# khaidoan25/prompt-tts

Hardware: NVIDIA B200
Metric: denoiser_train_codec_frames_per_sec (higher is better)
Workload: dtype bf16

## Files before the change

prompt_tts_b200/csrc/gemm_tcgen05.cu:

```cuda
#include <stdlib.h>

#include <mutex>

#include "tc_common.cuh"

namespace tc {
EncodeTiledFn get_encode_fn() {
  static EncodeTiledFn fn = nullptr;
  static std::once_flag once;
  std::call_once(once, [] {
    void* f = nullptr;
    cudaDriverEntryPointQueryResult qres;
    if (cudaGetDriverEntryPoint("cuTensorMapEncodeTiled", &f, cudaEnableDefault, &qres) == cudaSuccess && qres == cudaDriverEntryPointSuccess)
      fn = reinterpret_cast<EncodeTiledFn>(f);
  });
  return fn;
}
}

namespace {
using namespace tc;

constexpr int BM = 128;
constexpr int BK = 64;
constexpr int A_STAGE_BYTES = BM * BK * 2;

struct alignas(64) KParams {
  CUtensorMap tmA[2];
  CUtensorMap tmB[2];
  CUtensorMap tmO;
  pt_segment_t seg[8];
  int nseg;
  int a_kmajor, b_kmajor;
  int a_batched[2], b_batched[2];
  int M, N, nz2, nz3;
  int mt, nt, tiles, work, streamk;
  int gm;
  int total_iters;
  void* out;
  int out_dtype;
  long long osm, osz2, osz3;
  float alpha;
  const float* bias;
  const float* bias_z2;
  const bf16* res;
  long long rsm, rsz2, rsz3;
  long long bz2_stride;
  long long osn;
  int out_t;
  int vec_red;
};

template <int BN, bool PAIR = false>
struct Cfg {
  static constexpr int BN_LOAD = PAIR ? BN / 2 : BN;
  static constexpr int BN_S = (BN_LOAD + 63) / 64 * 64;
  static constexpr int B_STAGE_BYTES = BN_S * BK * 2;
  static constexpr int STAGE_BYTES = A_STAGE_BYTES + B_STAGE_BYTES;
  static constexpr int CTAS_PER_SM = (BN <= 128 && !PAIR) ? 2 : 1;
  static constexpr int EPI_WARPS = CTAS_PER_SM == 1 ? 8 : 4;
  static constexpr int EPI_SPLIT = EPI_WARPS / 4;
  static constexpr int THREADS = 64 + 32 * EPI_WARPS;
  static constexpr int EPI_COLS = 32;
#ifndef PT_EPI_BUFS
#define PT_EPI_BUFS 1
#endif
  static constexpr int EPI_BUFS = CTAS_PER_SM == 1 ? PT_EPI_BUFS : 1;
  static constexpr int EPI_BF16_BYTES = EPI_WARPS * EPI_BUFS * 32 * EPI_COLS * 2;
  static constexpr int EPI_F32_BYTES = EPI_WARPS * 32 * 17 * 4;
  static constexpr int EPI_BYTES = EPI_BF16_BYTES > EPI_F32_BYTES ? EPI_BF16_BYTES : EPI_F32_BYTES;
  static constexpr int F32_COLS = 16;
  static constexpr int BAR_BYTES = 512;
  static constexpr int BIAS_BYTES = 1024;
  static constexpr int AUX_BYTES = 1024  + BAR_BYTES + BIAS_BYTES + EPI_BYTES;
  static constexpr int STAGES_FIT = (227 * 1024 / CTAS_PER_SM - AUX_BYTES) / STAGE_BYTES;
  static constexpr int STAGES = STAGES_FIT > 8 ? 8 : STAGES_FIT;
  static constexpr int SMEM_BYTES = STAGES * STAGE_BYTES + AUX_BYTES;
  static constexpr int TMEM_COLS = 2 * BN <= 128 ? 128 : (2 * BN <= 256 ? 256 : 512);
};

struct Sched {
  int total_iters, streamk, cursor, end, stride;
  __device__ __forceinline__ Sched(const KParams& p, int mc) {
    total_iters = p.total_iters;
    streamk = p.streamk;
    const int nclu = (int)gridDim.x / mc, clu = (int)blockIdx.x / mc;
    if (streamk) {
      const int per = (p.work + nclu - 1) / nclu;
      cursor = min(p.work, clu * per);
      end = min(p.work, cursor + per);
      stride = 0;
    } else {
      cursor = clu;
      end = p.tiles;
      stride = nclu;
    }
  }
  __device__ __forceinline__ bool next(int& tile, int& it_begin, int& it_end) {
    if (cursor >= end) return false;
    if (streamk) {
      tile = cursor / total_iters;
      it_begin = cursor - tile * total_iters;
      it_end = min(total_iters, it_begin + (end - cursor));
      cursor += it_end - it_begin;
    } else {
      tile = cursor;
      it_begin = 0;
      it_end = total_iters;
      cursor += stride;
    }
    return true;
  }
};

template <int BN, int MC, bool PAIR>
__global__ void __launch_bounds__(Cfg<BN, PAIR>::THREADS, Cfg<BN, PAIR>::CTAS_PER_SM) gemm_kernel(const __grid_constant__ KParams p) {
  using C = Cfg<BN, PAIR>;
  static_assert(!PAIR || MC == 2, "a CTA pair is a cluster of two");
  const int crank = MC > 1 ? (int)cluster_ctarank() : 0;
  extern __shared__ uint8_t smem_raw[];
  const uint32_t smem_base = (smem_u32(smem_raw) + 1023u) & ~1023u;
  uint8_t* sgen = smem_raw + (smem_base - smem_u32(smem_raw));
  const uint32_t bar_base = smem_base + C::STAGES * C::STAGE_BYTES;
  auto full_bar = [&](int s) { return bar_base + 8u * s; };
  auto empty_bar = [&](int s) { return bar_base + 8u * (C::STAGES + s); };
  auto tmem_full_bar = [&](int a) { return bar_base + 8u * (2 * C::STAGES + a); };
  auto tmem_empty_bar = [&](int a) { return bar_base + 8u * (2 * C::STAGES + 2 + a); };
  const uint32_t tmem_slot = bar_base + 8u * (2 * C::STAGES + 4);
  float* sbias = reinterpret_cast<float*>(sgen + C::STAGES * C::STAGE_BYTES + C::BAR_BYTES);
  uint8_t* sepi = sgen + C::STAGES * C::STAGE_BYTES + C::BAR_BYTES + C::BIAS_BYTES;

  const int warp = threadIdx.x >> 5;
  const int lane = threadIdx.x & 31;

  if (warp == 0 && lane == 0) {
    asm volatile("prefetch.tensormap [%0];" ::"l"(reinterpret_cast<uint64_t>(&p.tmA[p.seg[0].a_idx])) : "memory");
    asm volatile("prefetch.tensormap [%0];" ::"l"(reinterpret_cast<uint64_t>(&p.tmB[p.seg[0].b_idx])) : "memory");
    for (int s = 0; s < C::STAGES; ++s) {
      mbar_init(full_bar(s), 1);
      mbar_init(empty_bar(s), PAIR ? 1 : MC);
    }
    for (int a = 0; a < 2; ++a) {
      mbar_init(tmem_full_bar(a), 1);
      mbar_init(tmem_empty_bar(a), PAIR ? 2 * C::EPI_WARPS : 32 * C::EPI_WARPS);
    }
    asm volatile("fence.mbarrier_init.release.cluster;" ::: "memory");
  }
  if (warp == 2) {
    if constexpr (PAIR) {
      asm volatile("tcgen05.alloc.cta_group::2.sync.aligned.shared::cta.b32 [%0], %1;" ::"r"(tmem_slot), "n"(C::TMEM_COLS) : "memory");
      asm volatile("tcgen05.relinquish_alloc_permit.cta_group::2.sync.aligned;" ::: "memory");
    } else {
      asm volatile("tcgen05.alloc.cta_group::1.sync.aligned.shared::cta.b32 [%0], %1;" ::"r"(tmem_slot), "n"(C::TMEM_COLS) : "memory");
      asm volatile("tcgen05.relinquish_alloc_permit.cta_group::1.sync.aligned;" ::: "memory");
    }
  }
  asm volatile("tcgen05.fence::before_thread_sync;" ::: "memory");
  __syncthreads();
  if (MC > 1) cluster_sync_all();
  asm volatile("tcgen05.fence::after_thread_sync;" ::: "memory");
  const uint32_t tmem_base = *reinterpret_cast<uint32_t*>(sgen + C::STAGES * C::STAGE_BYTES + 8 * (2 * C::STAGES + 4));

  auto decode = [&](int tile, int& m0, int& n0, int& z2, int& z3) {
    const int per_z = p.mt * p.nt;
    int r = tile / per_z;
    const int t = tile - r * per_z;
    const int span = p.gm * p.nt;
    const int grp = t / span;
    const int first = grp * p.gm;
    const int gsz = min(p.gm, p.mt - first);
    const int q = t - grp * span;
    const int mt = first + q % gsz;
    const int nt = q / gsz;
    m0 = (mt * MC + crank) * BM;
    n0 = nt * BN;
    z2 = r % p.nz2;
    z3 = r / p.nz2;
  };

  Sched sched(p, MC);
  int tile, it_begin, it_end;

  if (warp == 0) {
    const bool leader = elect_one();
    const uint32_t tx_own = A_STAGE_BYTES + (p.b_kmajor ? C::BN_LOAD * BK * 2 : C::B_STAGE_BYTES);
    const uint32_t tx_bytes = PAIR ? 2 * tx_own : tx_own;
    const uint32_t full0_leader = PAIR ? mapa_u32(full_bar(0), 0) : 0;
    int s = 0;
    uint32_t ph = 1;
    while (sched.next(tile, it_begin, it_end)) {
      int m0, n0, z2, z3;
      decode(tile, m0, n0, z2, z3);
      int seg = 0, rep = 0, kb = 0, skip = it_begin;
      while (true) {
        const int nkb = (p.seg[seg].nk + BK - 1) / BK;
        const int cnt = nkb * p.seg[seg].nrep;
        if (skip < cnt) {
          rep = skip / nkb;
          kb = skip % nkb;
          break;
        }
        skip -= cnt;
        ++seg;
      }
      for (int it = it_begin; it < it_end; ++it) {
        mbar_wait(empty_bar(s), ph);
        const pt_segment_t& sg = p.seg[seg];
        if (PAIR && leader) {
          if (crank == 0) mbar_expect_tx(full_bar(s), tx_bytes);
          const uint32_t sa = smem_base + s * C::STAGE_BYTES;
          const uint32_t sb = sa + A_STAGE_BYTES;
          const uint32_t fb = full0_leader + 8u * s;
          const CUtensorMap* ta = &p.tmA[sg.a_idx];
          const CUtensorMap* tb = &p.tmB[sg.b_idx];
          const int bz2 = sg.rep_is_batch ? (sg.rep_c2_0 + rep) : z2;
          const int a2 = p.a_batched[sg.a_idx] ? bz2 : 0, a3 = p.a_batched[sg.a_idx] ? z3 : 0;
          const int b2 = p.b_batched[sg.b_idx] ? bz2 : 0, b3 = p.b_batched[sg.b_idx] ? z3 : 0;
          const int ka = sg.a_k0 + kb * BK, kbb = sg.b_k0 + z2 * sg.b_k0_z2 + kb * BK;
          const int nb0 = n0 + sg.b_mn_shift + crank * C::BN_LOAD;
          if (p.a_kmajor) {
            tma_load_4d_pair(sa, ta, fb, ka, m0 + sg.a_mn_shift, a2, a3);
          } else {
#pragma unroll
            for (int j = 0; j < BM / 64; ++j) tma_load_4d_pair(sa + j * (BK * 128), ta, fb, m0 + sg.a_mn_shift + j * 64, ka, a2, a3);
          }
          if (p.b_kmajor) {
            tma_load_4d_pair(sb, tb, fb, kbb, nb0, b2, b3);
          } else {
#pragma unroll
            for (int j = 0; j < C::BN_S / 64; ++j) tma_load_4d_pair(sb + j * (BK * 128), tb, fb, nb0 + j * 64, kbb, b2, b3);
          }
        } else if (leader) {
          mbar_expect_tx(full_bar(s), tx_bytes);
          const uint32_t sa = smem_base + s * C::STAGE_BYTES;
          const uint32_t sb = sa + A_STAGE_BYTES;
          const CUtensorMap* ta = &p.tmA[sg.a_idx];
          const CUtensorMap* tb = &p.tmB[sg.b_idx];
          const int bz2 = sg.rep_is_batch ? (sg.rep_c2_0 + rep) : z2;
          const int a2 = p.a_batched[sg.a_idx] ? bz2 : 0, a3 = p.a_batched[sg.a_idx] ? z3 : 0;
          const int b2 = p.b_batched[sg.b_idx] ? bz2 : 0, b3 = p.b_batched[sg.b_idx] ? z3 : 0;
          const int ka = sg.a_k0 + kb * BK, kbb = sg.b_k0 + z2 * sg.b_k0_z2 + kb * BK;
          if (p.a_kmajor) {
            tma_load_4d(sa, ta, full_bar(s), ka, m0 + sg.a_mn_shift, a2, a3);
          } else {
#pragma unroll
            for (int j = 0; j < BM / 64; ++j) tma_load_4d(sa + j * (BK * 128), ta, full_bar(s), m0 + sg.a_mn_shift + j * 64, ka, a2, a3);
          }
          if (MC == 1) {
            if (p.b_kmajor) {
              tma_load_4d(sb, tb, full_bar(s), kbb, n0 + sg.b_mn_shift, b2, b3);
            } else {
#pragma unroll
              for (int j = 0; j < C::BN_S / 64; ++j) tma_load_4d(sb + j * (BK * 128), tb, full_bar(s), n0 + sg.b_mn_shift + j * 64, kbb, b2, b3);
            }
          } else {
            constexpr int HB = BN / MC;
            if (p.b_kmajor) {
              tma_load_4d_mc(sb + crank * (HB * 128), tb, full_bar(s), kbb, n0 + sg.b_mn_shift + crank * HB, b2, b3, (uint16_t)((1 << MC) - 1));
            } else {
#pragma unroll
              for (int j = 0; j < HB / 64; ++j) {
                const int jj = crank * (HB / 64) + j;
                tma_load_4d_mc(sb + jj * (BK * 128), tb, full_bar(s), n0 + sg.b_mn_shift + jj * 64, kbb, b2, b3, (uint16_t)((1 << MC) - 1));
              }
            }
          }
        }
        const int nkb = (sg.nk + BK - 1) / BK;
        if (++kb == nkb) {
          kb = 0;
          if (++rep == sg.nrep) {
            rep = 0;
            ++seg;
          }
        }
        if (++s == C::STAGES) s = 0, ph ^= 1;
      }
    }
  } else if (warp == 1 && (!PAIR || crank == 0)) {
    const bool leader = elect_one();
    const uint32_t idesc = idesc_f16(p.a_kmajor ? 0 : 1, p.b_kmajor ? 0 : 1, BN, PAIR ? 2 * BM : BM);
    const uint32_t a_lbo = p.a_kmajor ? 0u : (uint32_t)(BK * 128), b_lbo = p.b_kmajor ? 0u : (uint32_t)(BK * 128);
    const uint32_t a_kstep = p.a_kmajor ? 2u : 128u, b_kstep = p.b_kmajor ? 2u : 128u;
    const uint64_t adesc0 = umma_desc(smem_base, a_lbo, 1024);
    const uint64_t bdesc0 = umma_desc(smem_base + A_STAGE_BYTES, b_lbo, 1024);
    int s = 0;
    uint32_t ph = 0;
    int segi = 0;
    while (sched.next(tile, it_begin, it_end)) {
      const int acc = segi & 1;
      mbar_wait(tmem_empty_bar(acc), ((segi >> 1) & 1) ^ 1);
      asm volatile("tcgen05.fence::after_thread_sync;" ::: "memory");
      const uint32_t dcol = tmem_base + (uint32_t)(acc * BN);
      for (int it = it_begin; it < it_end; ++it) {
        mbar_wait(full_bar(s), ph);
        asm volatile("tcgen05.fence::after_thread_sync;" ::: "memory");
        if (leader) {
          const uint64_t ad = adesc0 + (uint64_t)(s * (C::STAGE_BYTES >> 4));
          const uint64_t bd = bdesc0 + (uint64_t)(s * (C::STAGE_BYTES >> 4));
          if constexpr (PAIR) {
#pragma unroll
            for (int k = 0; k < BK / 16; ++k)
              umma_f16_pair(dcol, ad + (uint64_t)(k * a_kstep), bd + (uint64_t)(k * b_kstep), idesc, (it > it_begin || k > 0) ? 1u : 0u);
            umma_commit_pair(empty_bar(s), (uint16_t)3);
            if (it == it_end - 1) umma_commit_pair(tmem_full_bar(acc), (uint16_t)3);
          } else {
#pragma unroll
            for (int k = 0; k < BK / 16; ++k)
              umma_f16(dcol, ad + (uint64_t)(k * a_kstep), bd + (uint64_t)(k * b_kstep), idesc, (it > it_begin || k > 0) ? 1u : 0u);
            if (MC == 1) umma_commit(empty_bar(s));
            else umma_commit_mc(empty_bar(s), (uint16_t)((1 << MC) - 1));
            if (it == it_end - 1) umma_commit(tmem_full_bar(acc));
          }
        }
        __syncwarp();
        if (++s == C::STAGES) s = 0, ph ^= 1;
      }
      ++segi;
    }
  } else if (warp >= 2) {
    const uint32_t tmem_empty_leader0 = PAIR ? mapa_u32(tmem_empty_bar(0), 0) : 0;
    auto release_acc = [&](int a) {
      asm volatile("tcgen05.fence::before_thread_sync;" ::: "memory");
      if constexpr (PAIR) {
        __syncwarp();
        if (lane == 0) mbar_arrive_cluster(tmem_empty_leader0 + 8u * a);
      } else {
        mbar_arrive(tmem_empty_bar(a));
      }
    };
    const int q = warp & 3;
    const int ew = warp - 2;
    const int half = ew >> 2;
    constexpr int ES = C::EPI_SPLIT;
    constexpr int ET = 32 * C::EPI_WARPS;
    const int et = threadIdx.x - 64;
    int segi = 0;
    int pc = 0;
    int staged_n0 = -1, staged_z2 = -1;
    while (sched.next(tile, it_begin, it_end)) {
      int m0, n0, z2, z3;
      decode(tile, m0, n0, z2, z3);
      const int acc = segi & 1;
      if (!p.out_t && (n0 != staged_n0 || (p.bias_z2 != nullptr && z2 != staged_z2))) {
        asm volatile("bar.sync 1, %0;" ::"n"(ET) : "memory");
        const float* bz = p.bias_z2 ? p.bias_z2 + (long long)z2 * p.bz2_stride : nullptr;
        for (int j = et; j < BN; j += ET) {
          const int n = n0 + j;
          float bsum = 0.f;
          if (n < p.N) {
            if (p.bias) bsum += __ldg(p.bias + n);
            if (bz) bsum += __ldg(bz + n);
          }
          sbias[j] = bsum;
        }
        asm volatile("bar.sync 1, %0;" ::"n"(ET) : "memory");
        staged_n0 = n0;
        staged_z2 = z2;
      }
      const uint32_t tbase = tmem_base + ((uint32_t)(q * 32) << 16) + (uint32_t)(acc * BN);
      const uint32_t full_parity = (segi >> 1) & 1;
      if (p.out_dtype == PT_OUT_BF16) {
        constexpr int CH = C::EPI_COLS;
        constexpr int NPASS = BN / CH;
        constexpr int NPH = (NPASS + ES - 1) / ES;
        constexpr int VPR = CH / 8;
        constexpr int RPI = 32 / VPR;
        constexpr int NIT = 32 / RPI;
        uint8_t* stg_base = sepi + ew * (C::EPI_BUFS * 32 * CH * 2);
        uint8_t* stg = stg_base + (pc & (C::EPI_BUFS - 1)) * (32 * CH * 2);
        auto cell = [&](int row, int chunk) { return stg + row * (CH * 2) + ((chunk ^ ((row >> 1) & 3)) << 4); };
        const int mw = m0 + q * 32;
        const int crow = lane / VPR, cvec = lane % VPR;
        const long long zoff_r = (long long)z2 * p.rsz2 + (long long)z3 * p.rsz3;
        const bool has_res = p.res != nullptr;
        const int last_c = min(NPASS, (p.N - n0 + CH - 1) / CH) - 1;
        const int last_k = last_c >= half ? (last_c - half) / ES : -1;
        uint32_t v[2][CH];
        bf16x8 rr[2][NIT];
        auto load_res = [&](int pass, bf16x8* dst) {
          if (p.out_t) {
            const int mb = mw + cvec * 8;
#pragma unroll
            for (int i = 0; i < NIT; ++i) {
              const int n = n0 + pass * CH + crow + i * RPI;
              if (n < p.N && mb < p.M) dst[i] = ld16(p.res + zoff_r + (long long)n * p.rsm + mb);
            }
            return;
          }
          const int nb = n0 + pass * CH + cvec * 8;
#pragma unroll
          for (int i = 0; i < NIT; ++i) {
            const int m = mw + crow + i * RPI;
            if (m < p.M && nb < p.N) dst[i] = ld16(p.res + zoff_r + (long long)m * p.rsm + nb);
          }
        };
        float brow = 0.f;
        if (p.out_t && mw + lane < p.M) {
          if (p.bias) brow += __ldg(p.bias + mw + lane);
          if (p.bias_z2) brow += __ldg(p.bias_z2 + (long long)z2 * p.bz2_stride + mw + lane);
        }
        if (has_res && last_k >= 0) load_res(half, rr[0]);
        mbar_wait(tmem_full_bar(acc), full_parity);
        asm volatile("tcgen05.fence::after_thread_sync;" ::: "memory");
        if (last_k < 0) {
          release_acc(acc);
        } else {
          tmem_ld32(tbase + (uint32_t)(half * CH), v[0]);
        }
#pragma unroll
        for (int k = 0; k < NPH; ++k) {
          const int c = half + k * ES;
          const int nb = n0 + c * CH;
          if (k <= last_k) {
            __syncwarp();
            asm volatile("tcgen05.wait::ld.sync.aligned;" ::: "memory");
            if (k < last_k) {
              tmem_ld32(tbase + (uint32_t)((c + ES) * CH), v[(k + 1) & 1]);
              if (has_res) load_res(c + ES, rr[(k + 1) & 1]);
            } else {
              release_acc(acc);
            }
            stg = stg_base + (pc & (C::EPI_BUFS - 1)) * (32 * CH * 2);
            if (lane == 0) {
              if (C::EPI_BUFS == 2) asm volatile("cp.async.bulk.wait_group.read 1;" ::: "memory");
              else asm volatile("cp.async.bulk.wait_group.read 0;" ::: "memory");
            }
            __syncwarp();
            if (has_res) {
#pragma unroll
              for (int i = 0; i < NIT; ++i) st16(cell(crow + i * RPI, cvec), rr[k & 1][i]);
              __syncwarp();
            }
            if (p.out_t) {
#pragma unroll
              for (int j = 0; j < CH; ++j) {
                bf16* cellp = reinterpret_cast<bf16*>(cell(j, lane >> 3)) + (lane & 7);
                float f = fmaf(__uint_as_float(v[k & 1][j]), p.alpha, brow);
                if (has_res) f += __bfloat162float(*cellp);
                *cellp = __float2bfloat16_rn(f);
              }
              fence_proxy_async_smem();
              __syncwarp();
              if (lane == 0) {
                tma_store_4d(&p.tmO, smem_u32(stg), mw, nb, z2, z3);
                tma_store_commit();
              }
              ++pc;
              continue;
            }
            const float* sb = sbias + c * CH;
#pragma unroll
            for (int g = 0; g < VPR; ++g) {
              const float4 b0 = *reinterpret_cast<const float4*>(sb + g * 8), b1 = *reinterpret_cast<const float4*>(sb + g * 8 + 4);
              const float bs[8] = {b0.x, b0.y, b0.z, b0.w, b1.x, b1.y, b1.z, b1.w};
              float f[8];
#pragma unroll
              for (int j = 0; j < 8; ++j) f[j] = fmaf(__uint_as_float(v[k & 1][g * 8 + j]), p.alpha, bs[j]);
              uint8_t* mine = cell(lane, g);
              if (has_res) {
                const bf16x8 t = ld16(mine);
#pragma unroll
                for (int h = 0; h < 4; ++h) {
                  const float2 u = bf2_to_f2(t.w[h]);
                  f[2 * h] += u.x;
                  f[2 * h + 1] += u.y;
                }
              }
              bf16x8 t;
#pragma unroll
              for (int h = 0; h < 4; ++h) t.w[h] = f2_to_bf2(f[2 * h], f[2 * h + 1]);
              st16(mine, t);
            }
            fence_proxy_async_smem();
            __syncwarp();
            if (lane == 0) {
              tma_store_4d(&p.tmO, smem_u32(stg), nb, mw, z2, z3);
              tma_store_commit();
            }
            ++pc;
          }
        }
      } else {
        const int m = m0 + q * 32 + lane;
        const bool m_ok = m < p.M;
        const long long out_off = (long long)z2 * p.osz2 + (long long)z3 * p.osz3 + (long long)m * p.osm;
        constexpr int FC = C::F32_COLS;
        constexpr int NCH = BN / FC;
        constexpr int NPH = (NCH + ES - 1) / ES;
        const int last_c = min(NCH, (p.N - n0 + FC - 1) / FC) - 1;
        const int last_k = last_c >= half ? (last_c - half) / ES : -1;
        uint32_t v[2][FC];
        mbar_wait(tmem_full_bar(acc), full_parity);
        asm volatile("tcgen05.fence::after_thread_sync;" ::: "memory");
        if (last_k < 0) {
          release_acc(acc);
        } else {
          tmem_ld16(tbase + (uint32_t)(half * FC), v[0]);
        }
        float* tile = reinterpret_cast<float*>(sepi) + ew * (32 * (FC + 1));
        const int mrow0 = m0 + q * 32;
        const long long zoff = (long long)z2 * p.osz2 + (long long)z3 * p.osz3;
#pragma unroll
        for (int k = 0; k < NPH; ++k) {
          const int c = half + k * ES;
          const int nb = n0 + c * FC;
          if (k <= last_k) {
            __syncwarp();
            asm volatile("tcgen05.wait::ld.sync.aligned;" ::: "memory");
            if (k < last_k) {
              tmem_ld16(tbase + (uint32_t)((c + ES) * FC), v[(k + 1) & 1]);
            } else {
              release_acc(acc);
            }
            float f[FC];
#pragma unroll
            for (int j = 0; j < FC; ++j) f[j] = fmaf(__uint_as_float(v[k & 1][j]), p.alpha, sbias[c * FC + j]);
            if (p.out_dtype == PT_OUT_F32) {
              if (m_ok) {
                float* o = reinterpret_cast<float*>(p.out) + out_off + nb;
#pragma unroll
                for (int g = 0; g < FC / 4; ++g) {
                  if (nb + g * 4 + 4 <= p.N) {
                    *reinterpret_cast<float4*>(o + g * 4) = make_float4(f[g * 4], f[g * 4 + 1], f[g * 4 + 2], f[g * 4 + 3]);
                  } else {
#pragma unroll
                    for (int j = 0; j < 4; ++j)
                      if (nb + g * 4 + j < p.N) o[g * 4 + j] = f[g * 4 + j];
                  }
                }
              }
            } else if (p.vec_red) {
              float* vt = reinterpret_cast<float*>(sepi) + ew * (32 * FC);
#pragma unroll
              for (int g = 0; g < FC / 4; ++g)
                *reinterpret_cast<float4*>(vt + lane * FC + ((g ^ ((lane >> 1) & 3)) << 2)) = make_float4(f[g * 4], f[g * 4 + 1], f[g * 4 + 2], f[g * 4 + 3]);
              __syncwarp();
              const int c4 = lane & 3, rsub = lane >> 2;
              const int n = nb + c4 * 4;
              if (n < p.N) {
                float* o = reinterpret_cast<float*>(p.out) + zoff + n;
#pragma unroll
                for (int it = 0; it < 4; ++it) {
                  const int r = it * 8 + rsub;
                  if (mrow0 + r < p.M) {
                    const float4 t = *reinterpret_cast<const float4*>(vt + r * FC + ((c4 ^ ((r >> 1) & 3)) << 2));
                    float* dst = o + (long long)(mrow0 + r) * p.osm;
                    if (n + 4 <= p.N) {
                      asm volatile("red.global.add.v4.f32 [%0], {%1, %2, %3, %4};" ::"l"(dst), "f"(t.x), "f"(t.y), "f"(t.z), "f"(t.w) : "memory");
                    } else {
                      const float tv[4] = {t.x, t.y, t.z, t.w};
#pragma unroll
                      for (int j = 0; j < 4; ++j)
                        if (n + j < p.N) atomicAdd(dst + j, tv[j]);
                    }
                  }
                }
              }
              __syncwarp();
            } else {
#pragma unroll
              for (int j = 0; j < FC; ++j) tile[lane * (FC + 1) + j] = f[j];
              __syncwarp();
              const int col = lane % FC, rsub = lane / FC;
              const int n = nb + col;
              if (n < p.N) {
                float* o = reinterpret_cast<float*>(p.out) + zoff + (long long)n * p.osn;
#pragma unroll 8
                for (int r = rsub; r < 32; r += 32 / FC) {
                  if (mrow0 + r < p.M) atomicAdd(o + (long long)(mrow0 + r) * p.osm, tile[r * (FC + 1) + col]);
                }
              }
            }
          }
        }
      }
      ++segi;
    }
    if (lane == 0) tma_store_wait_all();
  }

  asm volatile("tcgen05.fence::before_thread_sync;" ::: "memory");
  __syncthreads();
  if (MC > 1) cluster_sync_all();
  if (warp == 2) {
    if constexpr (PAIR) asm volatile("tcgen05.dealloc.cta_group::2.sync.aligned.b32 %0, %1;" ::"r"(tmem_base), "n"(C::TMEM_COLS) : "memory");
    else asm volatile("tcgen05.dealloc.cta_group::1.sync.aligned.b32 %0, %1;" ::"r"(tmem_base), "n"(C::TMEM_COLS) : "memory");
  }
}

int encode_operand(CUtensorMap* tm, const pt_operand_t& op, int box_rows_kmajor, const char* name) {
  EncodeTiledFn fn = get_encode_fn();
  if (!fn) {
    pt_set_error("cuTensorMapEncodeTiled not available from the driver");
    return PT_ECUDA;
  }
  PT_REQUIRE(op.ptr != nullptr, "gemm operand %s: null pointer", name);
  PT_REQUIRE((reinterpret_cast<uintptr_t>(op.ptr) & 15) == 0, "gemm operand %s: base not 16-byte aligned", name);
  PT_REQUIRE(op.stride[0] == 1, "gemm operand %s: dim[0] must be contiguous", name);
  cuuint64_t dims[4], strides[3];
  cuuint32_t box[4] = {64, 1, 1, 1}, estr[4] = {1, 1, 1, 1};
  for (int i = 0; i < 4; ++i) {
    PT_REQUIRE(op.dim[i] >= 1 && op.dim[i] < (1ll << 31), "gemm operand %s: dim[%d]=%lld out of range", name, i, (long long)op.dim[i]);
    dims[i] = (cuuint64_t)op.dim[i];
  }
  for (int i = 1; i < 4; ++i) {
    long long st = op.stride[i];
    if (op.dim[i] == 1 && (st <= 0 || (st % 8) != 0)) st = 8;
    PT_REQUIRE(st > 0 && st % 8 == 0, "gemm operand %s: stride[%d]=%lld must be a positive multiple of 8 elements", name, i, st);
    strides[i - 1] = (cuuint64_t)st * 2;
  }
  box[1] = op.kmajor ? (cuuint32_t)box_rows_kmajor : 64u;
  CUresult r = fn(tm, CU_TENSOR_MAP_DATA_TYPE_BFLOAT16, 4, const_cast<void*>(op.ptr), dims, strides, box, estr,
                  CU_TENSOR_MAP_INTERLEAVE_NONE, CU_TENSOR_MAP_SWIZZLE_128B, CU_TENSOR_MAP_L2_PROMOTION_L2_256B,
                  CU_TENSOR_MAP_FLOAT_OOB_FILL_NONE);
  if (r != CUDA_SUCCESS) {
    pt_set_error("cuTensorMapEncodeTiled(%s) failed: CUresult %d (dims %lld,%lld,%lld,%lld strides %lld,%lld,%lld box %u,%u)", name, (int)r,
                 (long long)dims[0], (long long)dims[1], (long long)dims[2], (long long)dims[3], (long long)strides[0],
                 (long long)strides[1], (long long)strides[2], box[0], box[1]);
    return PT_ECUDA;
  }
  return PT_OK;
}

int encode_output(CUtensorMap* tm, const pt_gemm_t* g) {
  EncodeTiledFn fn = get_encode_fn();
  if (!fn) {
    pt_set_error("cuTensorMapEncodeTiled not available from the driver");
    return PT_ECUDA;
  }
  PT_REQUIRE((reinterpret_cast<uintptr_t>(g->out) & 15) == 0, "pt_gemm: bf16 output base not 16-byte aligned");
  const long long ext[4] = {g->out_transposed ? g->M : g->N, g->out_transposed ? g->N : g->M, g->nz2, g->nz3};
  const long long str[4] = {1, g->out_stride_m, g->out_stride_z2, g->out_stride_z3};
  cuuint64_t dims[4], strides[3];
  for (int i = 0; i < 4; ++i) dims[i] = (cuuint64_t)ext[i];
  for (int i = 1; i < 4; ++i) {
    long long st = str[i];
    if (ext[i] == 1 && (st <= 0 || (st % 8) != 0)) st = 8;
    PT_REQUIRE(st > 0 && st % 8 == 0, "pt_gemm: bf16 output stride[%d]=%lld must be a positive multiple of 8 elements", i, st);
    strides[i - 1] = (cuuint64_t)st * 2;
  }
  cuuint32_t box[4] = {32, 32, 1, 1}, estr[4] = {1, 1, 1, 1};
  CUresult r = fn(tm, CU_TENSOR_MAP_DATA_TYPE_BFLOAT16, 4, g->out, dims, strides, box, estr, CU_TENSOR_MAP_INTERLEAVE_NONE,
                  CU_TENSOR_MAP_SWIZZLE_64B, CU_TENSOR_MAP_L2_PROMOTION_NONE, CU_TENSOR_MAP_FLOAT_OOB_FILL_NONE);
  if (r != CUDA_SUCCESS) {
    pt_set_error("cuTensorMapEncodeTiled(out) failed: CUresult %d (dims %lld,%lld,%lld,%lld strides %lld,%lld,%lld)", (int)r, ext[0], ext[1],
                 ext[2], ext[3], (long long)strides[0], (long long)strides[1], (long long)strides[2]);
    return PT_ECUDA;
  }
  return PT_OK;
}

template <int BN, int MC, bool PAIR = false>
int launch(const KParams& kp, dim3 grid, cudaStream_t st) {
  using CF = Cfg<BN, PAIR>;
  PT_ONCE_PER_DEVICE(cudaFuncSetAttribute(gemm_kernel<BN, MC, PAIR>, cudaFuncAttributeMaxDynamicSharedMemorySize, CF::SMEM_BYTES));
  if (MC == 1) {
    gemm_kernel<BN, MC, PAIR><<<grid, CF::THREADS, CF::SMEM_BYTES, st>>>(kp);
  } else {
    cudaLaunchConfig_t cfg = {};
    cfg.gridDim = grid;
    cfg.blockDim = dim3(CF::THREADS, 1, 1);
    cfg.dynamicSmemBytes = CF::SMEM_BYTES;
    cfg.stream = st;
    cudaLaunchAttribute attr[1];
    attr[0].id = cudaLaunchAttributeClusterDimension;
    attr[0].val.clusterDim.x = MC;
    attr[0].val.clusterDim.y = 1;
    attr[0].val.clusterDim.z = 1;
    cfg.attrs = attr;
    cfg.numAttrs = 1;
    static int max_clusters = 0;
    if (!max_clusters) {
      int n = 0;
      cudaLaunchConfig_t q = cfg;
      q.gridDim = dim3((unsigned)(pt_num_sms_physical() / MC * MC), 1, 1);
      if (cudaOccupancyMaxActiveClusters(&n, gemm_kernel<BN, MC, PAIR>, &q) != cudaSuccess || n < 1) {
        (void)cudaGetLastError();
        n = pt_num_sms_physical() / MC;
      }
      max_clusters = n;
      if (getenv("PT_GEMM_DEBUG")) fprintf(stderr, "[pt_gemm] BN=%d cluster=%d pair=%d: %d clusters resident at once\n", BN, MC, (int)PAIR, n);
    }
    if ((int)grid.x / MC > max_clusters) cfg.gridDim = dim3((unsigned)(max_clusters * MC), 1, 1);
    PT_CUDA_OK(cudaLaunchKernelEx(&cfg, gemm_kernel<BN, MC, PAIR>, kp));
  }
  PT_LAUNCH_CHECK();
  return PT_OK;
}

}

static thread_local int g_last_tile = 0;
extern "C" int pt_gemm_last_tile(void) { return g_last_tile; }

extern "C" int pt_gemm(const pt_gemm_t* g, void* stream) {
  PT_REQUIRE(g != nullptr, "pt_gemm: null descriptor");
  PT_REQUIRE(g->nseg >= 1 && g->nseg <= 8, "pt_gemm: nseg=%d", g->nseg);
  PT_REQUIRE(g->M >= 1 && g->N >= 1, "pt_gemm: M=%d N=%d", g->M, g->N);
  PT_REQUIRE(g->nz2 >= 1 && g->nz3 >= 1, "pt_gemm: bad batch extents");
  PT_REQUIRE(g->out != nullptr, "pt_gemm: null output");
  if (g->out_dtype == PT_OUT_BF16) {
    PT_REQUIRE((g->out_transposed ? g->M : g->N) % 8 == 0 && g->out_stride_m % 8 == 0 && g->out_stride_z2 % 8 == 0 && g->out_stride_z3 % 8 == 0 &&
                   (reinterpret_cast<uintptr_t>(g->out) & 15) == 0,
               "pt_gemm: bf16 output needs N (M if transposed), strides multiples of 8 and a 16-byte aligned base (M=%d N=%d)", g->M, g->N);
  } else if (g->out_dtype == PT_OUT_F32) {
    PT_REQUIRE(g->out_stride_m % 4 == 0 && g->out_stride_z2 % 4 == 0 && g->out_stride_z3 % 4 == 0 &&
                   (reinterpret_cast<uintptr_t>(g->out) & 15) == 0,
               "pt_gemm: f32 output needs N, strides multiples of 4 (N=%d)", g->N);
  } else {
    PT_REQUIRE(g->out_dtype == PT_OUT_F32_ATOMIC_ADD, "pt_gemm: out_dtype=%d", g->out_dtype);
  }
  if (g->residual) {
    PT_REQUIRE((g->out_transposed ? g->M : g->N) % 8 == 0 && g->res_stride_m % 8 == 0 && g->res_stride_z2 % 8 == 0 && g->res_stride_z3 % 8 == 0 &&
                   (reinterpret_cast<uintptr_t>(g->residual) & 15) == 0,
               "pt_gemm: residual alignment");
  }

  KParams kp;
  memset(&kp, 0, sizeof(kp));
  bool a_used[2] = {false, false}, b_used[2] = {false, false};
  long long total = 0;
  for (int i = 0; i < g->nseg; ++i) {
    const pt_segment_t& s = g->seg[i];
    PT_REQUIRE(s.a_idx >= 0 && s.a_idx < 2 && s.b_idx >= 0 && s.b_idx < 2, "pt_gemm: segment %d operand index", i);
    PT_REQUIRE(s.nk >= 1 && s.nrep >= 1, "pt_gemm: segment %d nk=%d nrep=%d", i, s.nk, s.nrep);
    a_used[s.a_idx] = true;
    b_used[s.b_idx] = true;
    kp.seg[i] = s;
    total += (long long)((s.nk + BK - 1) / BK) * s.nrep;
  }
  PT_REQUIRE(total < (1ll << 30), "pt_gemm: too many k iterations");
  const int a0 = a_used[0] ? 0 : 1, b0 = b_used[0] ? 0 : 1;
  kp.a_kmajor = g->a[a0].kmajor;
  kp.b_kmajor = g->b[b0].kmajor;
  for (int i = 0; i < 2; ++i) {
    if (a_used[i]) PT_REQUIRE(g->a[i].kmajor == kp.a_kmajor, "pt_gemm: A operands must share one majorness");
    if (b_used[i]) PT_REQUIRE(g->b[i].kmajor == kp.b_kmajor, "pt_gemm: B operands must share one majorness");
  }

  const bool streamk = g->out_dtype == PT_OUT_F32_ATOMIC_ADD;
  PT_REQUIRE(!streamk || (g->bias == nullptr && g->bias_z2 == nullptr && g->residual == nullptr),
             "pt_gemm: PT_OUT_F32_ATOMIC_ADD outputs are scheduled stream-K and take no bias/residual");
  int bn = g->block_n & ~1;
  bool table_no_cluster = false;
  const bool allow_cluster_arg = (g->block_n & 1) == 0;
  const long long mt = (g->M + BM - 1) / BM;
  const long long zz = (long long)g->nz2 * g->nz3;
  const int sms = pt_num_sms();
  if (g->block_n == 0) {
    struct TileRow { int M, N, K, zz, nseg, ak, bk, od, res, bn; };
    static const TileRow table[] = {
#include "gemm_tile_table.inc"
        {0, 0, 0, 0, 0, 0, 0, 0, 0, 0}};
    static const bool no_table = getenv("PT_GEMM_NO_TABLE") != nullptr;
    if (!no_table) {
      long long ktot = 0;
      for (int s = 0; s < g->nseg; ++s) ktot += (long long)g->seg[s].nk * g->seg[s].nrep;
      for (const TileRow& r : table)
        if (r.M == g->M && r.N == g->N && r.K == ktot && r.zz == zz && r.nseg == g->nseg && r.ak == kp.a_kmajor && r.bk == kp.b_kmajor &&
            r.od == g->out_dtype && r.res == (g->residual != nullptr)) {
          bn = r.bn & ~1;
          table_no_cluster = (r.bn & 1) != 0;
          break;
        }
    }
  }
  const bool allow_cluster = allow_cluster_arg && !table_no_cluster;
  if (bn == 0) {
    const int cand[6] = {256, 224, 192, 128, 64, 160};
    const double cyc[6] = {mt >= 2 && allow_cluster && !streamk ? 780.0 : 800.0, 730.0, 660.0, 430.0, streamk ? 416.0 : 260.0, 640.0};
    double best = 1e300;
    for (int i = 0; i < 6; ++i) {
      const int c = cand[i];
      const long long tiles_c = mt * ((g->N + c - 1) / c) * zz;
      double cost;
      if (streamk) {
        const double slots_c = (double)sms * (c <= 128 ? 2 : 1);
        cost = (double)tiles_c * (double)total * cyc[i] / sms + 0.65 * ((double)tiles_c + slots_c) * c;
      } else {
        cost = (double)((tiles_c + sms - 1) / sms) * ((double)total * cyc[i] + 500.0);
      }
      if (cost < best * 0.97) {
        best = cost;
        bn = c;
      }
    }
  }
  PT_REQUIRE(bn == 64 || bn == 96 || bn == 128 || bn == 160 || bn == 192 || bn == 224 || bn == 256, "pt_gemm: block_n=%d", bn);
  PT_REQUIRE(bn != 96 || kp.b_kmajor, "pt_gemm: block_n = 96 needs a K-major B operand");
  PT_REQUIRE(!g->out_transposed || (g->out_dtype == PT_OUT_BF16 && g->M % 8 == 0), "pt_gemm: out_transposed needs a bf16 output and M %% 8 == 0 (M=%d)", g->M);

  const int mc = (bn == 256 && mt >= 2 && allow_cluster && !streamk) ? 2 : 1;
  static const bool no_pair = getenv("PT_GEMM_NO_PAIR") != nullptr;
  const bool pair = mc == 2 && !no_pair && (mt % 2 == 0 || mt >= 8) && total >= 16;
  for (int i = 0; i < 2; ++i) {
    if (a_used[i]) {
      int r = encode_operand(&kp.tmA[i], g->a[i], BM, i ? "A1" : "A0");
      if (r) return r;
      kp.a_batched[i] = g->a[i].batched;
    }
    if (b_used[i]) {
      int r = encode_operand(&kp.tmB[i], g->b[i], bn / mc, i ? "B1" : "B0");
      if (r) return r;
      kp.b_batched[i] = g->b[i].batched;
    }
  }
  if (g->out_dtype == PT_OUT_BF16) {
    if (int r = encode_output(&kp.tmO, g)) return r;
  }
  kp.nseg = g->nseg;
  kp.M = g->M;
  kp.N = g->N;
  kp.nz2 = g->nz2;
  kp.nz3 = g->nz3;
  kp.total_iters = (int)total;
  const long long nt = (g->N + bn - 1) / bn;
  const long long mtg = (mt + mc - 1) / mc;
  const long long tiles = mtg * nt * zz;
  PT_REQUIRE(tiles * total < (1ll << 31), "pt_gemm: work space too large");
  kp.mt = (int)mtg;
  kp.nt = (int)nt;
  kp.tiles = (int)tiles;
  kp.work = (int)(tiles * total);
  kp.streamk = streamk ? 1 : 0;
  {
    static const bool no_group = getenv("PT_GEMM_NO_GROUP") != nullptr;
    const long long resident = (long long)sms * (bn <= 128 ? 2 : 1) / mc;
    long long gm = (resident + nt / 2) / nt;
    if (gm < 1) gm = 1;
    if (gm > mtg || no_group || streamk) gm = mtg;
    kp.gm = (int)gm;
  }
  kp.out = g->out;
  kp.out_dtype = g->out_dtype;
  kp.osm = g->out_stride_m;
  kp.osz2 = g->out_stride_z2;
  kp.osz3 = g->out_stride_z3;
  kp.alpha = g->alpha;
  kp.bias = g->bias;
  kp.bias_z2 = g->bias_z2;
  kp.res = reinterpret_cast<const bf16*>(g->residual);
  kp.rsm = g->res_stride_m;
  kp.rsz2 = g->res_stride_z2;
  kp.rsz3 = g->res_stride_z3;
  kp.bz2_stride = g->bias_z2_stride ? g->bias_z2_stride : g->N;
  kp.osn = g->out_stride_n ? g->out_stride_n : 1;
  kp.out_t = g->out_transposed ? 1 : 0;
  PT_REQUIRE(kp.osn == 1 || g->out_dtype == PT_OUT_F32_ATOMIC_ADD, "pt_gemm: out_stride_n needs PT_OUT_F32_ATOMIC_ADD");
  kp.vec_red = (g->out_dtype == PT_OUT_F32_ATOMIC_ADD && kp.osn == 1 && g->out_stride_m % 4 == 0 && g->out_stride_z2 % 4 == 0 &&
                g->out_stride_z3 % 4 == 0 && (reinterpret_cast<uintptr_t>(g->out) & 15) == 0 && !getenv("PT_GEMM_SCALAR_RED"))
                   ? 1 : 0;

  const long long slots = (long long)sms * (bn <= 128 ? 2 : 1) / mc;
  long long G = streamk ? (kp.work / 4 > 0 ? kp.work / 4 : 1) : tiles;
  if (G > slots) G = slots;
  dim3 grid((unsigned)(G * mc), 1, 1);
  cudaStream_t st = reinterpret_cast<cudaStream_t>(stream);
  g_last_tile = bn | (bn == 256 && mc == 1 ? 1 : 0);
  switch (bn) {
    case 64: return launch<64, 1>(kp, grid, st);
    case 96: return launch<96, 1>(kp, grid, st);
    case 128: return launch<128, 1>(kp, grid, st);
    case 160: return launch<160, 1>(kp, grid, st);
    case 192: return launch<192, 1>(kp, grid, st);
    case 224: return launch<224, 1>(kp, grid, st);
    default: return mc == 2 ? (pair ? launch<256, 2, true>(kp, grid, st) : launch<256, 2>(kp, grid, st)) : launch<256, 1>(kp, grid, st);
  }
}
```

prompt_tts_b200/csrc/tc_common.cuh:

```cuda
#pragma once
#include <cuda.h>

#include "common.cuh"

namespace tc {

__device__ __forceinline__ uint32_t smem_u32(const void* p) { return (uint32_t)__cvta_generic_to_shared(p); }

__device__ __forceinline__ bool elect_one() {
  uint32_t pred;
  asm volatile(
      "{\n\t.reg .pred p;\n\t"
      "elect.sync _|p, 0xffffffff;\n\t"
      "selp.u32 %0, 1, 0, p;\n\t}"
      : "=r"(pred));
  return pred != 0;
}

__device__ __forceinline__ void mbar_init(uint32_t bar, uint32_t count) {
  asm volatile("mbarrier.init.shared::cta.b64 [%0], %1;" ::"r"(bar), "r"(count) : "memory");
}
__device__ __forceinline__ void mbar_arrive(uint32_t bar) {
  asm volatile("mbarrier.arrive.shared::cta.b64 _, [%0];" ::"r"(bar) : "memory");
}
__device__ __forceinline__ void mbar_expect_tx(uint32_t bar, uint32_t bytes) {
  asm volatile("mbarrier.arrive.expect_tx.shared::cta.b64 _, [%0], %1;" ::"r"(bar), "r"(bytes) : "memory");
}
__device__ __forceinline__ void mbar_wait(uint32_t bar, uint32_t parity) {
  uint32_t done = 0;
  uint32_t spins = 0;
  while (true) {
    asm volatile(
        "{\n\t.reg .pred p;\n\t"
        "mbarrier.try_wait.parity.shared::cta.b64 p, [%1], %2;\n\t"
        "selp.u32 %0, 1, 0, p;\n\t}"
        : "=r"(done)
        : "r"(bar), "r"(parity)
        : "memory");
    if (done) break;
#ifdef PT_MBAR_WATCH
    if (spins == (1u << 20)) PT_MBAR_WATCH(bar, parity);
#endif
    if (++spins > (1u << 22)) __trap();
  }
}

__device__ __forceinline__ void tma_load_4d(uint32_t dst, const CUtensorMap* tm, uint32_t bar, int c0, int c1, int c2, int c3) {
  asm volatile(
      "cp.async.bulk.tensor.4d.shared::cluster.global.mbarrier::complete_tx::bytes [%0], [%1, {%3, %4, %5, %6}], [%2];"
      ::"r"(dst), "l"(reinterpret_cast<uint64_t>(tm)), "r"(bar), "r"(c0), "r"(c1), "r"(c2), "r"(c3)
      : "memory");
}

__device__ __forceinline__ void tma_store_4d(const CUtensorMap* tm, uint32_t src, int c0, int c1, int c2, int c3) {
  asm volatile("cp.async.bulk.tensor.4d.global.shared::cta.bulk_group [%0, {%2, %3, %4, %5}], [%1];" ::"l"(reinterpret_cast<uint64_t>(tm)),
               "r"(src), "r"(c0), "r"(c1), "r"(c2), "r"(c3)
               : "memory");
}
__device__ __forceinline__ void tma_store_commit() { asm volatile("cp.async.bulk.commit_group;" ::: "memory"); }
__device__ __forceinline__ void tma_store_wait_read() { asm volatile("cp.async.bulk.wait_group.read 0;" ::: "memory"); }
__device__ __forceinline__ void tma_store_wait_all() { asm volatile("cp.async.bulk.wait_group 0;" ::: "memory"); }
__device__ __forceinline__ void fence_proxy_async_smem() { asm volatile("fence.proxy.async.shared::cta;" ::: "memory"); }

__device__ __forceinline__ void tma_load_4d_mc(uint32_t dst, const CUtensorMap* tm, uint32_t bar, int c0, int c1, int c2, int c3, uint16_t mask) {
  asm volatile(
      "cp.async.bulk.tensor.4d.shared::cluster.global.mbarrier::complete_tx::bytes.multicast::cluster [%0], [%1, {%3, %4, %5, %6}], [%2], %7;"
      ::"r"(dst), "l"(reinterpret_cast<uint64_t>(tm)), "r"(bar), "r"(c0), "r"(c1), "r"(c2), "r"(c3), "h"(mask)
      : "memory");
}

__device__ __forceinline__ uint64_t umma_desc(uint32_t saddr, uint32_t lbo_bytes, uint32_t sbo_bytes) {
  uint64_t d = 0;
  d |= (uint64_t)((saddr >> 4) & 0x3FFF);
  d |= (uint64_t)((lbo_bytes >> 4) & 0x3FFF) << 16;
  d |= (uint64_t)((sbo_bytes >> 4) & 0x3FFF) << 32;
  d |= 1ull << 46;
  d |= 2ull << 61;
  return d;
}

__device__ __forceinline__ void umma_f16(uint32_t tmem_d, uint64_t adesc, uint64_t bdesc, uint32_t idesc, uint32_t accumulate) {
  asm volatile(
      "{\n\t.reg .pred p;\n\t"
      "setp.ne.b32 p, %4, 0;\n\t"
      "tcgen05.mma.cta_group::1.kind::f16 [%0], %1, %2, %3, p;\n\t}"
      ::"r"(tmem_d), "l"(adesc), "l"(bdesc), "r"(idesc), "r"(accumulate)
      : "memory");
}
__device__ __forceinline__ void umma_f16_ts(uint32_t tmem_d, uint32_t tmem_a, uint64_t bdesc, uint32_t idesc, uint32_t accumulate) {
  asm volatile(
      "{\n\t.reg .pred p;\n\t"
      "setp.ne.b32 p, %4, 0;\n\t"
      "tcgen05.mma.cta_group::1.kind::f16 [%0], [%1], %2, %3, p;\n\t}"
      ::"r"(tmem_d), "r"(tmem_a), "l"(bdesc), "r"(idesc), "r"(accumulate)
      : "memory");
}
__device__ __forceinline__ void umma_commit(uint32_t bar) {
  asm volatile("tcgen05.commit.cta_group::1.mbarrier::arrive::one.shared::cluster.b64 [%0];" ::"r"(bar) : "memory");
}

__device__ __forceinline__ void umma_commit_mc(uint32_t bar, uint16_t mask) {
  asm volatile("tcgen05.commit.cta_group::1.mbarrier::arrive::one.shared::cluster.multicast::cluster.b64 [%0], %1;" ::"r"(bar), "h"(mask) : "memory");
}
__device__ __forceinline__ uint32_t mapa_u32(uint32_t addr, uint32_t rank) {
  uint32_t r;
  asm volatile("mapa.shared::cluster.u32 %0, %1, %2;" : "=r"(r) : "r"(addr), "r"(rank));
  return r;
}
__device__ __forceinline__ void tma_load_4d_pair(uint32_t dst, const CUtensorMap* tm, uint32_t bar_cluster, int c0, int c1, int c2, int c3) {
  asm volatile(
      "cp.async.bulk.tensor.4d.cta_group::2.shared::cluster.global.mbarrier::complete_tx::bytes [%0], [%1, {%3, %4, %5, %6}], [%2];"
      ::"r"(dst), "l"(reinterpret_cast<uint64_t>(tm)), "r"(bar_cluster), "r"(c0), "r"(c1), "r"(c2), "r"(c3)
      : "memory");
}
__device__ __forceinline__ void mbar_arrive_cluster(uint32_t bar_cluster) {
  asm volatile("mbarrier.arrive.release.cluster.shared::cluster.b64 _, [%0];" ::"r"(bar_cluster) : "memory");
}
__device__ __forceinline__ void umma_f16_pair(uint32_t tmem_d, uint64_t adesc, uint64_t bdesc, uint32_t idesc, uint32_t accumulate) {
  asm volatile(
      "{\n\t.reg .pred p;\n\t"
      "setp.ne.b32 p, %4, 0;\n\t"
      "tcgen05.mma.cta_group::2.kind::f16 [%0], %1, %2, %3, p;\n\t}"
      ::"r"(tmem_d), "l"(adesc), "l"(bdesc), "r"(idesc), "r"(accumulate)
      : "memory");
}
__device__ __forceinline__ void umma_commit_pair(uint32_t bar, uint16_t mask) {
  asm volatile("tcgen05.commit.cta_group::2.mbarrier::arrive::one.shared::cluster.multicast::cluster.b64 [%0], %1;" ::"r"(bar), "h"(mask) : "memory");
}

__device__ __forceinline__ uint32_t cluster_ctarank() {
  uint32_t r;
  asm volatile("mov.u32 %0, %%cluster_ctarank;" : "=r"(r));
  return r;
}
__device__ __forceinline__ void cluster_sync_all() {
  asm volatile("barrier.cluster.arrive.release.aligned;" ::: "memory");
  asm volatile("barrier.cluster.wait.acquire.aligned;" ::: "memory");
}

__device__ __forceinline__ void tmem_st16(uint32_t taddr, const uint32_t* v) {
  asm volatile(
      "tcgen05.st.sync.aligned.32x32b.x16.b32 [%0], "
      "{%1, %2, %3, %4, %5, %6, %7, %8, %9, %10, %11, %12, %13, %14, %15, %16};"
      ::"r"(taddr), "r"(v[0]), "r"(v[1]), "r"(v[2]), "r"(v[3]), "r"(v[4]), "r"(v[5]), "r"(v[6]), "r"(v[7]), "r"(v[8]), "r"(v[9]), "r"(v[10]),
        "r"(v[11]), "r"(v[12]), "r"(v[13]), "r"(v[14]), "r"(v[15])
      : "memory");
}
__device__ __forceinline__ void tmem_wait_st() { asm volatile("tcgen05.wait::st.sync.aligned;" ::: "memory"); }

__device__ __forceinline__ void tmem_ld32(uint32_t taddr, uint32_t* v) {
  asm volatile(
      "tcgen05.ld.sync.aligned.32x32b.x32.b32 "
      "{%0, %1, %2, %3, %4, %5, %6, %7, %8, %9, %10, %11, %12, %13, %14, %15, "
      "%16, %17, %18, %19, %20, %21, %22, %23, %24, %25, %26, %27, %28, %29, %30, %31}, [%32];"
      : "=r"(v[0]), "=r"(v[1]), "=r"(v[2]), "=r"(v[3]), "=r"(v[4]), "=r"(v[5]), "=r"(v[6]), "=r"(v[7]), "=r"(v[8]),
        "=r"(v[9]), "=r"(v[10]), "=r"(v[11]), "=r"(v[12]), "=r"(v[13]), "=r"(v[14]), "=r"(v[15]), "=r"(v[16]),
        "=r"(v[17]), "=r"(v[18]), "=r"(v[19]), "=r"(v[20]), "=r"(v[21]), "=r"(v[22]), "=r"(v[23]), "=r"(v[24]),
        "=r"(v[25]), "=r"(v[26]), "=r"(v[27]), "=r"(v[28]), "=r"(v[29]), "=r"(v[30]), "=r"(v[31])
      : "r"(taddr)
      : "memory");
}
__device__ __forceinline__ void tmem_ld16(uint32_t taddr, uint32_t* v) {
  asm volatile(
      "tcgen05.ld.sync.aligned.32x32b.x16.b32 "
      "{%0, %1, %2, %3, %4, %5, %6, %7, %8, %9, %10, %11, %12, %13, %14, %15}, [%16];"
      : "=r"(v[0]), "=r"(v[1]), "=r"(v[2]), "=r"(v[3]), "=r"(v[4]), "=r"(v[5]), "=r"(v[6]), "=r"(v[7]), "=r"(v[8]),
        "=r"(v[9]), "=r"(v[10]), "=r"(v[11]), "=r"(v[12]), "=r"(v[13]), "=r"(v[14]), "=r"(v[15])
      : "r"(taddr)
      : "memory");
}

__device__ __forceinline__ uint32_t idesc_f16(int a_mn_major, int b_mn_major, int n, int m) {
  return (1u << 4) | (1u << 7) | (1u << 10) | ((uint32_t)a_mn_major << 15) | ((uint32_t)b_mn_major << 16) | ((uint32_t)(n >> 3) << 17) |
         ((uint32_t)(m >> 4) << 24);
}

typedef CUresult (*EncodeTiledFn)(CUtensorMap*, CUtensorMapDataType, cuuint32_t, void*, const cuuint64_t*, const cuuint64_t*,
                                  const cuuint32_t*, const cuuint32_t*, CUtensorMapInterleave, CUtensorMapSwizzle,
                                  CUtensorMapL2promotion, CUtensorMapFloatOOBfill);
EncodeTiledFn get_encode_fn();

}
```

prompt_tts_b200/engine.py:

```python
from __future__ import annotations

import os
from typing import Callable, Dict, List, Optional, Sequence, Tuple

import torch

from . import ops
from .ops import BF16, F32, OUT_BF16, OUT_F32, OUT_F32_ATOMIC_ADD



class Var:
    __slots__ = ("data", "grad", "owned", "needs_grad")

    def __init__(self, data: torch.Tensor, needs_grad: bool = True):
        self.data = data
        self.grad: Optional[torch.Tensor] = None
        self.owned = False
        self.needs_grad = needs_grad


class SideLane:

    def __init__(self, device):
        self.stream = torch.cuda.Stream(device)
        self.keep: List[torch.Tensor] = []
        self.dirty = False

    def run(self, fn: Callable[[], None], keep: Sequence[torch.Tensor] = ()) -> None:
        self.stream.wait_stream(torch.cuda.current_stream())
        with torch.cuda.stream(self.stream):
            fn()
        self.keep.extend(keep)
        self.dirty = True

    def join(self) -> None:
        if self.dirty:
            torch.cuda.current_stream().wait_stream(self.stream)
            self.dirty = False
            self.keep.clear()


SIDE_LANE = os.environ.get("PT_SIDE_LANE", "0") == "1"


class PackCache:

    def __init__(self):
        self._d: Dict[tuple, Tuple[tuple, torch.Tensor]] = {}
        self.static: Dict[tuple, list] = {}
        self.lane: Optional[SideLane] = None
        self.epoch = 0

    def add_static(self, kind: str, params: Sequence[torch.Tensor], view: torch.Tensor, refresh: Optional[Callable[[], None]]) -> None:
        key = (kind,) + tuple(id(p) for p in params)
        self.static[key] = [tuple(p._version for p in params), view, refresh, list(params)]

    def get(self, params: Sequence[torch.Tensor], kind: str) -> torch.Tensor:
        key = (kind,) + tuple(id(p) for p in params)
        st = self.static.get(key)
        if st is not None:
            ver = tuple(p._version for p in params)
            if ver != st[0]:
                if st[2] is not None:
                    st[2]()
                st[0] = ver
            return st[1]
        ver = (self.epoch,) + tuple((p._version, p.data_ptr()) for p in params)
        hit = self._d.get(key)
        capturing = torch.cuda.is_current_stream_capturing() if params[0].is_cuda else False
        if hit is not None and hit[0] == ver and not capturing:
            return hit[1]
        prev = hit[1] if hit is not None else None
        if kind == "conv":
            (w,) = params
            if not w.is_contiguous():
                raise ops._lib.PtError("conv weight is a non-contiguous view (optimiser-managed) but has no static bf16 shadow")
            out = ops.pack_conv_weight(w.detach(), out=prev)
        elif kind == "bias":
            if len(params) == 1:
                out = params[0].detach()
            else:
                out = torch.cat([p.detach() for p in params], out=prev) if prev is not None else torch.cat([p.detach() for p in params])
        else:
            rows = sum(p.shape[0] for p in params)
            K = params[0].numel() // params[0].shape[0]
            out = prev if prev is not None else torch.empty(rows, K, dtype=BF16, device=params[0].device)
            r = 0
            for p in params:
                ops.cast_bf16(p.detach().reshape(p.shape[0], K), out[r:r + p.shape[0]])
                r += p.shape[0]
        self._d[key] = (ver, out)
        return out


class Tape:
    def __init__(self, cache: PackCache, recording: bool = True):
        self.cache = cache
        self.recording = recording
        self.bwd: List[Callable[[], None]] = []
        self.pgrads: Dict[int, torch.Tensor] = {}
        self.params: Dict[int, torch.Tensor] = {}
        self.post: List[Callable[[], None]] = []
        self.pgrad_order: List[Tuple[Sequence[torch.Tensor], torch.Tensor, str]] = []
        self.grad_alloc: Optional[Callable[[Sequence[torch.Tensor], str], Optional[torch.Tensor]]] = None
        self.on_ready: Optional[Callable[[List[Tuple[Sequence[torch.Tensor], torch.Tensor, str]]], None]] = None
        self.kv_cache: Optional[Dict[int, "Var"]] = None
        self.kv_group: Dict[int, Tuple["Var", int, int]] = {}

    def record(self, fn: Callable[[], None]) -> None:
        if self.recording:
            self.bwd.append(fn)

    def _register(self, params: Sequence[torch.Tensor], kind: str, buf: torch.Tensor) -> None:
        if kind == "plain":
            (p,) = params
            self.pgrads[id(p)] = buf.view(p.shape)
            self.params[id(p)] = p
        elif kind == "conv":
            (p,) = params
            Co, Ci, k = p.shape
            packed = buf.view(Co, k, Ci)
            g = packed.permute(0, 2, 1)
            g._pt_buf = packed
            self.pgrads[id(p)] = g
            self.params[id(p)] = p
        else:
            rows = sum(p.shape[0] for p in params)
            K = params[0].numel() // params[0].shape[0]
            cat = buf.view(rows, K)
            r = 0
            for p in params:
                v = cat[r:r + p.shape[0]].view(p.shape)
                v._pt_buf = cat
                self.pgrads[id(p)] = v
                self.params[id(p)] = p
                r += p.shape[0]

    def _grad_buf(self, params: Sequence[torch.Tensor], kind: str) -> torch.Tensor:
        g = self.pgrads.get(id(params[0]))
        if g is None:
            n = sum(p.numel() for p in params)
            buf = self.grad_alloc(params, kind) if self.grad_alloc is not None else None
            if buf is None:
                buf = torch.zeros(n, dtype=F32, device=params[0].device)
            self._register(params, kind, buf)
            self.pgrad_order.append((list(params), buf, kind))
            g = self.pgrads[id(params[0])]
        return getattr(g, "_pt_buf", g)

    def rebind(self, params: Sequence[torch.Tensor], kind: str, buf: torch.Tensor) -> None:
        self._register(params, kind, buf)

    def pgrad(self, p: torch.Tensor) -> torch.Tensor:
        return self._grad_buf([p], "plain")

    def pgrad_cat(self, params: Sequence[torch.Tensor]) -> torch.Tensor:
        return self._grad_buf(params, "cat")

    def pgrad_conv(self, p: torch.Tensor) -> torch.Tensor:
        return self._grad_buf([p], "conv")

    def side_colsum(self, x2d: torch.Tensor, out: torch.Tensor) -> None:
        if not SIDE_LANE or not x2d.is_cuda:
            ops.colsum(x2d, out)
            return
        if self.cache.lane is None:
            self.cache.lane = SideLane(x2d.device)
        self.cache.lane.run(lambda: ops.colsum(x2d, out, lite=True), keep=(x2d, out))

    def join_side(self) -> None:
        if self.cache.lane is not None:
            self.cache.lane.join()

    def backward(self) -> None:
        done = 0
        for fn in reversed(self.bwd):
            fn()
            if self.on_ready is not None and len(self.pgrad_order) > done:
                self.on_ready(self.pgrad_order[done:])
                done = len(self.pgrad_order)
        self.bwd = []
        self.join_side()
        for fn in self.post:
            fn()
        self.post = []


def accum(v: Var, g: torch.Tensor, owned: bool = True) -> None:
    if not v.needs_grad:
        return
    if v.grad is None:
        v.grad, v.owned = g, owned
    elif v.owned:
        ops.add_(v.grad, g, out=v.grad)
    else:
        v.grad = ops.add_(v.grad, g)
        v.owned = True


def _wgrad_gemm(dy2d_op, x2d_op, seg, N: int, K: int, out: torch.Tensor, out_stride_m: int) -> None:
    ops.gemm([dy2d_op], [x2d_op], [seg], N, K, out, out_strides=(out_stride_m, 0, 0), out_mode=OUT_F32_ATOMIC_ADD)


def linear(tape: Tape, x: Var, wparams: Sequence[torch.Tensor], bias: Optional[Sequence[torch.Tensor]] = None,
           residual: Optional[Var] = None, out_f32: bool = False) -> Var:
    xd = x.data
    K = xd.shape[-1]
    x2 = xd.reshape(-1, K)
    M = x2.shape[0]
    wp = tape.cache.get(wparams, "lin")
    N = wp.shape[0]
    out = torch.empty(xd.shape[:-1] + (N,), dtype=F32 if out_f32 else BF16, device=xd.device)
    res = residual.data.reshape(M, N) if residual is not None else None
    ops.gemm([ops.operand(x2, True)], [ops.operand(wp, True)], [ops.segment(K)], M, N, out,
             out_mode=OUT_F32 if out_f32 else OUT_BF16, bias=tape.cache.get(bias, "bias") if bias is not None else None, residual=res)
    y = Var(out)

    def bwd():
        dy = y.grad
        if dy is None:
            return
        if out_f32:
            dy = ops.cast_bf16(dy)
        dy2 = dy.reshape(M, N)
        if bias is not None:
            tape.side_colsum(dy2, tape.pgrad_cat(bias) if len(bias) > 1 else tape.pgrad(bias[0]))
        gw = (tape.pgrad_cat(wparams) if len(wparams) > 1 else tape.pgrad(wparams[0])).view(N, K)
        _wgrad_gemm(ops.operand(dy2, False), ops.operand(x2, False), ops.segment(M), N, K, gw, K)
        if x.needs_grad:
            dx = torch.empty_like(x2) if (x.grad is None or not x.owned) else x.grad.reshape(M, K)
            prev = x.grad.reshape(M, K) if x.grad is not None else None
            ops.gemm([ops.operand(dy2, True)], [ops.operand(wp, False)], [ops.segment(N)], M, K, dx, residual=prev)
            x.grad, x.owned = dx.view(xd.shape), True
        if residual is not None:
            accum(residual, dy.view(residual.data.shape) if not out_f32 else dy.view(residual.data.shape), owned=False)

    tape.record(bwd)
    return y


class TimeShift:

    def __init__(self, proj: torch.Tensor, dproj: Optional[torch.Tensor], offset: int):
        self.proj, self.dproj, self.offset = proj, dproj, offset


CONV_SWAP = os.environ.get("PT_CONV_NO_SWAP") is None


def _swap_tile(L: int, rows: int) -> int:
    if not CONV_SWAP or rows % 128 != 0 or L > 96:
        return 0
    bn = 64 if L <= 64 else 96
    return bn if L / bn > L / 128 + 0.08 else 0


def conv3(tape: Tape, x: Var, wparam: torch.Tensor, bias: torch.Tensor, stride: int = 1,
          tshift: Optional[TimeShift] = None, residual: Optional[Var] = None) -> Var:
    xd = x.data
    B, L, Ci = xd.shape
    wp = tape.cache.get([wparam], "conv")
    Co = wp.shape[0]
    Lo = L if stride == 1 else (L - 1) // 2 + 1
    out = torch.empty(B, Lo, Co, dtype=BF16, device=xd.device)
    if stride == 1:
        a_ops = [ops.operand(xd, True, batched=True)]
        taps = [(0, t - 1) for t in range(3)]
    else:
        a_ops = [ops.operand(xd[:, 0::2], True, batched=True), ops.operand(xd[:, 1::2], True, batched=True)]
        taps = [(1, -1), (0, 0), (1, 0)]
    segs = [ops.segment(Ci, a_idx=ai, a_shift=sh, b_k0=t * Ci) for t, (ai, sh) in enumerate(taps)]
    bz2 = tshift.proj[:, tshift.offset:] if tshift is not None else None
    sw = _swap_tile(L, Co) if stride == 1 else 0
    if sw:
        segs_w = [ops.segment(Ci, a_k0=t * Ci, b_shift=t - 1) for t in range(3)]
        ops.gemm([ops.operand(wp, True)], a_ops, segs_w, Co, Lo, out, out_strides=(Co, Lo * Co, 0), nz2=B,
                 bias=bias.detach(), bias_z2=bz2, bias_z2_stride=tshift.proj.stride(0) if tshift is not None else 0,
                 residual=residual.data if residual is not None else None, res_strides=(Co, Lo * Co, 0), block_n=sw, out_transposed=True)
    else:
        ops.gemm(a_ops, [ops.operand(wp, True)], segs, Lo, Co, out, out_strides=(Co, Lo * Co, 0), nz2=B,
                 bias=bias.detach(), bias_z2=bz2, bias_z2_stride=tshift.proj.stride(0) if tshift is not None else 0,
                 residual=residual.data if residual is not None else None, res_strides=(Co, Lo * Co, 0))
    y = Var(out)

    def bwd():
        dy = y.grad
        if dy is None:
            return
        tape.side_colsum(dy.view(B * Lo, Co), tape.pgrad(bias))
        if tshift is not None and tshift.dproj is not None:
            ops.batch_colsum(dy, tshift.dproj[:, tshift.offset:], tshift.dproj.stride(0))
        g3 = tape.pgrad_conv(wparam)
        dy_op = ops.operand(dy, False, batched=True)
        if stride == 1:
            seg = ops.segment(Lo, b_k0=-1, b_k0_z2=1, nrep=B, rep_is_batch=True)
            ops.gemm([dy_op], [ops.operand(xd, False, batched=True)], [seg], Co, Ci, g3, out_strides=(3 * Ci, Ci, 0), nz2=3,
                     out_mode=OUT_F32_ATOMIC_ADD)
        else:
            for t, (ai, sh) in enumerate(taps):
                xs = xd[:, 0::2] if ai == 0 else xd[:, 1::2]
                seg = ops.segment(Lo, b_k0=sh, nrep=B, rep_is_batch=True)
                ops.gemm([dy_op], [ops.operand(xs, False, batched=True)], [seg], Co, Ci, g3[:, t],
                         out_strides=(3 * Ci, 0, 0), out_mode=OUT_F32_ATOMIC_ADD)
        if x.needs_grad:
            dy_k = ops.operand(dy, True, batched=True)
            wp_mn = ops.operand(wp, False)
            if stride == 1:
                own = x.grad is not None and x.owned
                dx = x.grad if own else torch.empty_like(xd)
                swx = _swap_tile(L, Ci)
                if swx:
                    segs_dx = [ops.segment(Co, a_shift=t * Ci, b_shift=1 - t) for t in range(3)]
                    ops.gemm([wp_mn], [dy_k], segs_dx, Ci, L, dx, out_strides=(Ci, L * Ci, 0), nz2=B,
                             residual=x.grad, res_strides=(Ci, L * Ci, 0), block_n=swx, out_transposed=True)
                else:
                    segs_dx = [ops.segment(Co, a_shift=1 - t, b_shift=t * Ci) for t in range(3)]
                    ops.gemm([dy_k], [wp_mn], segs_dx, L, Ci, dx, out_strides=(Ci, L * Ci, 0), nz2=B,
                             residual=x.grad, res_strides=(Ci, L * Ci, 0))
                x.grad, x.owned = dx, True
            else:
                dx = torch.empty_like(xd)
                ev, od = dx[:, 0::2], dx[:, 1::2]
                ops.gemm([dy_k], [wp_mn], [ops.segment(Co, b_shift=Ci)], ev.shape[1], Ci, ev, out_strides=(2 * Ci, L * Ci, 0), nz2=B)
                if od.shape[1] > 0:
                    ops.gemm([dy_k], [wp_mn], [ops.segment(Co, a_shift=1, b_shift=0), ops.segment(Co, a_shift=0, b_shift=2 * Ci)],
                             od.shape[1], Ci, od, out_strides=(2 * Ci, L * Ci, 0), nz2=B)
                accum(x, dx, owned=True)
        if residual is not None:
            accum(residual, dy, owned=False)

    tape.record(bwd)
    return y


def groupnorm(tape: Tape, x: Var, gamma: torch.Tensor, beta: torch.Tensor, eps: float, act: bool, groups: int = 32) -> Var:
    yd, stats = ops.groupnorm_fwd(x.data, gamma.detach(), beta.detach(), groups, eps, act)
    y = Var(yd)

    def bwd():
        if y.grad is None:
            return
        if not x.needs_grad:
            ops.groupnorm_bwd(y.grad, x.data, stats, gamma.detach(), beta.detach(), tape.pgrad(gamma), tape.pgrad(beta), groups, act)
            return
        prev = x.grad
        dx = ops.groupnorm_bwd(y.grad, x.data, stats, gamma.detach(), beta.detach(), tape.pgrad(gamma), tape.pgrad(beta), groups, act,
                               dx_add=prev, out=prev if (prev is not None and x.owned) else None)
        x.grad, x.owned = dx, True

    tape.record(bwd)
    return y


def layernorm(tape: Tape, x: Var, gamma: torch.Tensor, beta: torch.Tensor, eps: float = 1e-5) -> Var:
    xd = x.data
    Cc = xd.shape[-1]
    x2 = xd.reshape(-1, Cc)
    yd, rs = ops.layernorm_fwd(x2, gamma.detach(), beta.detach(), eps)
    y = Var(yd.view(xd.shape))

    def bwd():
        if y.grad is None:
            return
        prev = x.grad.reshape(-1, Cc) if x.grad is not None else None
        dx = ops.layernorm_bwd(y.grad.reshape(-1, Cc), x2, rs, gamma.detach(), tape.pgrad(gamma), tape.pgrad(beta), dx_add=prev)
        if x.needs_grad:
            x.grad, x.owned = dx.view(xd.shape), True

    tape.record(bwd)
    return y


def attention_core(tape: Tape, q_src: Var, q_off: int, kv_src: Var, k_off: int, v_off: int, heads: int, C: int,
                   shared_kv: bool = False) -> Var:
    qd, kvd = q_src.data, kv_src.data
    B, Lq, _ = qd.shape
    d = C // heads
    scale = d ** -0.5
    qv, kv_, vv = qd[:, :, q_off:q_off + C], kvd[:, :, k_off:k_off + C], kvd[:, :, v_off:v_off + C]
    o = torch.empty(B, Lq, C, dtype=BF16, device=qd.device)
    lse = torch.empty(B, heads, Lq, dtype=F32, device=qd.device)
    ops.attn_fwd(qv, kv_, vv, o, lse, heads, d, scale)
    y = Var(o)

    def bwd():
        do = y.grad
        if do is None:
            return
        same = q_src is kv_src
        dq_buf = torch.empty_like(qd)
        if shared_kv:
            if kv_src.grad is None:
                kv_src.grad, kv_src.owned = torch.empty_like(kvd), True
            dkv_buf = kv_src.grad
        else:
            dkv_buf = dq_buf if same else torch.empty_like(kvd)
        ops.attn_bwd(qv, kv_, vv, o, lse, do, dq_buf[:, :, q_off:q_off + C], dkv_buf[:, :, k_off:k_off + C],
                     dkv_buf[:, :, v_off:v_off + C], heads, d, scale)
        accum(q_src, dq_buf, owned=True)
        if not same and not shared_kv:
            accum(kv_src, dkv_buf, owned=True)

    tape.record(bwd)
    return y


def geglu(tape: Tape, u: Var) -> Var:
    ud = u.data
    u2 = ud.reshape(-1, ud.shape[-1])
    y = Var(ops.geglu_fwd(u2).view(ud.shape[:-1] + (ud.shape[-1] // 2,)))

    def bwd():
        if y.grad is None:
            return
        accum(u, ops.geglu_bwd(y.grad.reshape(-1, ud.shape[-1] // 2), u2).view(ud.shape), owned=True)

    tape.record(bwd)
    return y


def add(tape: Tape, a: Var, b: Var) -> Var:
    y = Var(ops.add_(a.data, b.data))

    def bwd():
        if y.grad is None:
            return
        accum(a, y.grad, owned=False)
        accum(b, y.grad, owned=False)

    tape.record(bwd)
    return y


def concat_channels(tape: Tape, a: Var, b: Var) -> Var:
    B, L, Ca = a.data.shape
    Cb = b.data.shape[2]
    out = torch.empty(B, L, Ca + Cb, dtype=BF16, device=a.data.device)
    ops.copy2d(a.data, Ca, out, Ca + Cb, B * L, Ca)
    ops.copy2d(b.data, Cb, out[:, :, Ca:], Ca + Cb, B * L, Cb)
    y = Var(out)

    def bwd():
        if y.grad is None:
            return
        g = y.grad
        ga = torch.empty_like(a.data)
        gb = torch.empty_like(b.data)
        ops.copy2d(g, Ca + Cb, ga, Ca, B * L, Ca)
        ops.copy2d(g[:, :, Ca:], Ca + Cb, gb, Cb, B * L, Cb)
        accum(a, ga, owned=True)
        accum(b, gb, owned=True)

    tape.record(bwd)
    return y


def upsample2(tape: Tape, x: Var) -> Var:
    y = Var(ops.upsample2_fwd(x.data))

    def bwd():
        if y.grad is None:
            return
        accum(x, ops.upsample2_bwd(y.grad), owned=True)

    tape.record(bwd)
    return y


def silu_f32(tape: Tape, x: Var) -> Var:
    y = Var(ops.silu_to_bf16(x.data))

    def bwd():
        if y.grad is None or not x.needs_grad:
            return
        g = ops.silu_bwd(x.data, ops.cast_f32(y.grad))
        if x.grad is None:
            x.grad, x.owned = g, True
        else:
            x.grad = x.grad + g

    tape.record(bwd)
    return y


class TapeFunction(torch.autograd.Function):

    @staticmethod
    def forward(ctx, runner, cache, n_in, *args):
        ins, params = args[:n_in], args[n_in:]
        need = any(ctx.needs_input_grad[3:])
        tape = Tape(cache, recording=need)
        outs, seed, in_grads = runner(tape, *ins)
        ctx.tape, ctx.seed, ctx.in_grads, ctx.n_in, ctx.params = tape, seed, in_grads, n_in, params
        ctx.mark_non_differentiable(*[o for o in outs if not o.is_floating_point()])
        return outs if len(outs) > 1 else outs[0]

    @staticmethod
    def backward(ctx, *gouts):
        tape = ctx.tape
        ctx.seed([g.contiguous() if g is not None else None for g in gouts])
        tape.backward()
        gin = ctx.in_grads()
        gparams = tuple(tape.pgrads.get(id(p)) if ctx.needs_input_grad[3 + ctx.n_in + i] else None for i, p in enumerate(ctx.params))
        ctx.tape = None
        return (None, None, None) + tuple(gin) + gparams


def get_cache(module) -> PackCache:
    c = module.__dict__.get("_pt_pack_cache")
    if c is None:
        c = PackCache()
        module.__dict__["_pt_pack_cache"] = c
    return c


def run_module(module, body, inputs, kinds, out_kind="ncl", multi=False):
    params = [p for p in module.parameters()]
    cache = get_cache(module)
    for t in inputs:
        if not t.is_cuda:
            raise ops._lib.PtError(f"{type(module).__name__}: inputs must be CUDA tensors; there is no CPU fallback")

    def runner(tape, *ins):
        vs = []
        for t, k in zip(ins, kinds):
            if k == "ncl":
                vs.append(Var(ops.ncl_to_nlc(t.detach().float().contiguous())))
            elif k == "blc":
                vs.append(Var(ops.cast_bf16(t.detach().float().contiguous())))
            elif k == "f32":
                vs.append(Var(t.detach().float().contiguous()))
            else:
                vs.append(t.detach())
        res = body(tape, *vs)
        yvs = list(res) if multi else [res]
        outs = tuple(ops.nlc_to_ncl(v.data) if out_kind == "ncl" else ops.cast_f32(v.data) for v in yvs)

        def seed(gouts):
            for v, g in zip(yvs, gouts):
                if g is None:
                    continue
                gg = ops.ncl_to_nlc(g.float().contiguous()) if out_kind == "ncl" else ops.cast_bf16(g.float().contiguous())
                accum(v, gg, owned=True)

        def in_grads():
            r = []
            for v, k in zip(vs, kinds):
                if k == "raw" or v.grad is None:
                    r.append(None)
                elif k == "ncl":
                    r.append(ops.nlc_to_ncl(v.grad))
                elif k == "blc":
                    r.append(ops.cast_f32(v.grad))
                else:
                    r.append(v.grad)
            return r

        return outs, seed, in_grads

    return TapeFunction.apply(runner, cache, len(inputs), *inputs, *params)
```

Before: 533,800.

## Use cluster launch control scheduling and overlap weight-grad GEMMs on side stream

Replaces the static persistent/stream-K scheduler in the tcgen05 GEMM with cluster-launch-control work stealing. The grid is now sized to the total number of work units, and resident CTAs cancel pending CTAs to pull more units, with stream-K split into roughly two units per slot. Separately, the Python engine makes the side stream always on and moves weight-gradient GEMMs and bias colsums onto it, retaining gradient tensors up to a byte cap. This aims to reduce tail imbalance and to overlap wgrad with dgrad work, at the cost of extra barriers, held memory and possible contention on the atomic adds.

```diff
diff --git a/prompt_tts_b200/csrc/gemm_tcgen05.cu b/prompt_tts_b200/csrc/gemm_tcgen05.cu
--- a/prompt_tts_b200/csrc/gemm_tcgen05.cu
+++ b/prompt_tts_b200/csrc/gemm_tcgen05.cu
@@ -34,7 +34,8 @@
   int a_kmajor, b_kmajor;
   int a_batched[2], b_batched[2];
   int M, N, nz2, nz3;
-  int mt, nt, tiles, work, streamk;
+  int mt, nt, work;
+  int unit_iters;
   int gm;
   int total_iters;
   void* out;
@@ -77,38 +78,23 @@
   static constexpr int STAGES = STAGES_FIT > 8 ? 8 : STAGES_FIT;
   static constexpr int SMEM_BYTES = STAGES * STAGE_BYTES + AUX_BYTES;
   static constexpr int TMEM_COLS = 2 * BN <= 128 ? 128 : (2 * BN <= 256 ? 256 : 512);
+  static constexpr int CLC_SLOTS = 8;
+  static constexpr int CLC_RESP_OFF = (8 * (2 * STAGES + 5 + 2 * CLC_SLOTS) + 15) / 16 * 16;
+  static_assert(CLC_RESP_OFF + 16 * CLC_SLOTS <= BAR_BYTES, "barrier region");
 };
 
-struct Sched {
-  int total_iters, streamk, cursor, end, stride;
-  __device__ __forceinline__ Sched(const KParams& p, int mc) {
-    total_iters = p.total_iters;
-    streamk = p.streamk;
-    const int nclu = (int)gridDim.x / mc, clu = (int)blockIdx.x / mc;
-    if (streamk) {
-      const int per = (p.work + nclu - 1) / nclu;
-      cursor = min(p.work, clu * per);
-      end = min(p.work, cursor + per);
-      stride = 0;
-    } else {
-      cursor = clu;
-      end = p.tiles;
-      stride = nclu;
-    }
-  }
-  __device__ __forceinline__ bool next(int& tile, int& it_begin, int& it_end) {
+struct UnitWalk {
+  int cursor, end;
+  __device__ __forceinline__ UnitWalk(const KParams& p, int unit) {
+    cursor = unit * p.unit_iters;
+    end = min(p.work, cursor + p.unit_iters);
+  }
+  __device__ __forceinline__ bool next(const KParams& p, int& tile, int& it_begin, int& it_end) {
     if (cursor >= end) return false;
-    if (streamk) {
-      tile = cursor / total_iters;
-      it_begin = cursor - tile * total_iters;
-      it_end = min(total_iters, it_begin + (end - cursor));
-      cursor += it_end - it_begin;
-    } else {
-      tile = cursor;
-      it_begin = 0;
-      it_end = total_iters;
-      cursor += stride;
-    }
+    tile = cursor / p.total_iters;
+    it_begin = cursor - tile * p.total_iters;
+    it_end = min(p.total_iters, it_begin + (end - cursor));
+    cursor += it_end - it_begin;
     return true;
   }
 };
@@ -127,6 +113,10 @@
   auto tmem_full_bar = [&](int a) { return bar_base + 8u * (2 * C::STAGES + a); };
   auto tmem_empty_bar = [&](int a) { return bar_base + 8u * (2 * C::STAGES + 2 + a); };
   const uint32_t tmem_slot = bar_base + 8u * (2 * C::STAGES + 4);
+  constexpr int R = C::CLC_SLOTS;
+  auto clc_full = [&](int i) { return bar_base + 8u * (2 * C::STAGES + 5 + i); };
+  auto clc_empty = [&](int i) { return bar_base + 8u * (2 * C::STAGES + 5 + R + i); };
+  auto clc_resp = [&](int i) { return bar_base + (uint32_t)C::CLC_RESP_OFF + 16u * i; };
   float* sbias = reinterpret_cast<float*>(sgen + C::STAGES * C::STAGE_BYTES + C::BAR_BYTES);
   uint8_t* sepi = sgen + C::STAGES * C::STAGE_BYTES + C::BAR_BYTES + C::BIAS_BYTES;
 
@@ -143,6 +133,10 @@
     for (int a = 0; a < 2; ++a) {
       mbar_init(tmem_full_bar(a), 1);
       mbar_init(tmem_empty_bar(a), PAIR ? 2 * C::EPI_WARPS : 32 * C::EPI_WARPS);
+    }
+    for (int i = 0; i < R; ++i) {
+      mbar_init(clc_full(i), 1);
+      mbar_init(clc_empty(i), MC * (1 + C::EPI_WARPS) + (PAIR ? 1 : MC));
     }
     asm volatile("fence.mbarrier_init.release.cluster;" ::: "memory");
   }
@@ -178,7 +172,21 @@
     z3 = r / p.nz2;
   };
 
-  Sched sched(p, MC);
+  const uint32_t clc_empty_rank0 = MC > 1 ? mapa_u32(clc_empty(0), 0) : clc_empty(0);
+  auto next_unit = [&](int j, int& unit) -> bool {
+    const int slot = j % R;
+    mbar_wait(clc_full(slot), (uint32_t)(j / R) & 1u);
+    const int x = clc_first_ctaid_x(clc_resp(slot));
+    __syncwarp();
+    if (lane == 0) {
+      if (MC > 1) mbar_arrive_cluster(clc_empty_rank0 + 8u * slot);
+      else mbar_arrive(clc_empty(slot));
+    }
+    if (x < 0) return false;
+    unit = x / MC;
+    return true;
+  };
+  const int first_unit = (int)blockIdx.x / MC;
   int tile, it_begin, it_end;
 
   if (warp == 0) {
@@ -188,94 +196,109 @@
     const uint32_t full0_leader = PAIR ? mapa_u32(full_bar(0), 0) : 0;
     int s = 0;
     uint32_t ph = 1;
-    while (sched.next(tile, it_begin, it_end)) {
-      int m0, n0, z2, z3;
-      decode(tile, m0, n0, z2, z3);
-      int seg = 0, rep = 0, kb = 0, skip = it_begin;
-      while (true) {
-        const int nkb = (p.seg[seg].nk + BK - 1) / BK;
-        const int cnt = nkb * p.seg[seg].nrep;
-        if (skip < cnt) {
-          rep = skip / nkb;
-          kb = skip % nkb;
-          break;
+    int unit = first_unit;
+    for (int j = 0;; ++j) {
+      if (leader) {
+        const int slot = j % R;
+        if (crank == 0) mbar_wait(clc_empty(slot), ((uint32_t)(j / R) & 1u) ^ 1u);
+        mbar_expect_tx(clc_full(slot), 16);
+        if (crank == 0) {
+          fence_proxy_async_smem();
+          clc_try_cancel<(MC > 1)>(clc_resp(slot), clc_full(slot));
         }
-        skip -= cnt;
-        ++seg;
       }
-      for (int it = it_begin; it < it_end; ++it) {
-        mbar_wait(empty_bar(s), ph);
-        const pt_segment_t& sg = p.seg[seg];
-        if (PAIR && leader) {
-          if (crank == 0) mbar_expect_tx(full_bar(s), tx_bytes);
-          const uint32_t sa = smem_base + s * C::STAGE_BYTES;
-          const uint32_t sb = sa + A_STAGE_BYTES;
-          const uint32_t fb = full0_leader + 8u * s;
-          const CUtensorMap* ta = &p.tmA[sg.a_idx];
-          const CUtensorMap* tb = &p.tmB[sg.b_idx];
-          const int bz2 = sg.rep_is_batch ? (sg.rep_c2_0 + rep) : z2;
-          const int a2 = p.a_batched[sg.a_idx] ? bz2 : 0, a3 = p.a_batched[sg.a_idx] ? z3 : 0;
-          const int b2 = p.b_batched[sg.b_idx] ? bz2 : 0, b3 = p.b_batched[sg.b_idx] ? z3 : 0;
-          const int ka = sg.a_k0 + kb * BK, kbb = sg.b_k0 + z2 * sg.b_k0_z2 + kb * BK;
-          const int nb0 = n0 + sg.b_mn_shift + crank * C::BN_LOAD;
-          if (p.a_kmajor) {
-            tma_load_4d_pair(sa, ta, fb, ka, m0 + sg.a_mn_shift, a2, a3);
-          } else {
-#pragma unroll
-            for (int j = 0; j < BM / 64; ++j) tma_load_4d_pair(sa + j * (BK * 128), ta, fb, m0 + sg.a_mn_shift + j * 64, ka, a2, a3);
-          }
-          if (p.b_kmajor) {
-            tma_load_4d_pair(sb, tb, fb, kbb, nb0, b2, b3);
-          } else {
-#pragma unroll
-            for (int j = 0; j < C::BN_S / 64; ++j) tma_load_4d_pair(sb + j * (BK * 128), tb, fb, nb0 + j * 64, kbb, b2, b3);
-          }
-        } else if (leader) {
-          mbar_expect_tx(full_bar(s), tx_bytes);
-          const uint32_t sa = smem_base + s * C::STAGE_BYTES;
-          const uint32_t sb = sa + A_STAGE_BYTES;
-          const CUtensorMap* ta = &p.tmA[sg.a_idx];
-          const CUtensorMap* tb = &p.tmB[sg.b_idx];
-          const int bz2 = sg.rep_is_batch ? (sg.rep_c2_0 + rep) : z2;
-          const int a2 = p.a_batched[sg.a_idx] ? bz2 : 0, a3 = p.a_batched[sg.a_idx] ? z3 : 0;
-          const int b2 = p.b_batched[sg.b_idx] ? bz2 : 0, b3 = p.b_batched[sg.b_idx] ? z3 : 0;
-          const int ka = sg.a_k0 + kb * BK, kbb = sg.b_k0 + z2 * sg.b_k0_z2 + kb * BK;
-          if (p.a_kmajor) {
-            tma_load_4d(sa, ta, full_bar(s), ka, m0 + sg.a_mn_shift, a2, a3);
-          } else {
-#pragma unroll
-            for (int j = 0; j < BM / 64; ++j) tma_load_4d(sa + j * (BK * 128), ta, full_bar(s), m0 + sg.a_mn_shift + j * 64, ka, a2, a3);
-          }
-          if (MC == 1) {
+      __syncwarp();
+      UnitWalk walk(p, unit);
+      while (walk.next(p, tile, it_begin, it_end)) {
+        int m0, n0, z2, z3;
+        decode(tile, m0, n0, z2, z3);
+        int seg = 0, rep = 0, kb = 0, skip = it_begin;
+        while (true) {
+          const int nkb = (p.seg[seg].nk + BK - 1) / BK;
+          const int cnt = nkb * p.seg[seg].nrep;
+          if (skip < cnt) {
+            rep = skip / nkb;
+            kb = skip % nkb;
+            break;
+          }
+          skip -= cnt;
+          ++seg;
+        }
+        for (int it = it_begin; it < it_end; ++it) {
+          mbar_wait(empty_bar(s), ph);
+          const pt_segment_t& sg = p.seg[seg];
+          if (PAIR && leader) {
+            if (crank == 0) mbar_expect_tx(full_bar(s), tx_bytes);
+            const uint32_t sa = smem_base + s * C::STAGE_BYTES;
+            const uint32_t sb = sa + A_STAGE_BYTES;
+            const uint32_t fb = full0_leader + 8u * s;
+            const CUtensorMap* ta = &p.tmA[sg.a_idx];
+            const CUtensorMap* tb = &p.tmB[sg.b_idx];
+            const int bz2 = sg.rep_is_batch ? (sg.rep_c2_0 + rep) : z2;
+            const int a2 = p.a_batched[sg.a_idx] ? bz2 : 0, a3 = p.a_batched[sg.a_idx] ? z3 : 0;
+            const int b2 = p.b_batched[sg.b_idx] ? bz2 : 0, b3 = p.b_batched[sg.b_idx] ? z3 : 0;
+            const int ka = sg.a_k0 + kb * BK, kbb = sg.b_k0 + z2 * sg.b_k0_z2 + kb * BK;
+            const int nb0 = n0 + sg.b_mn_shift + crank * C::BN_LOAD;
+            if (p.a_kmajor) {
+              tma_load_4d_pair(sa, ta, fb, ka, m0 + sg.a_mn_shift, a2, a3);
+            } else {
+  #pragma unroll
+              for (int j = 0; j < BM / 64; ++j) tma_load_4d_pair(sa + j * (BK * 128), ta, fb, m0 + sg.a_mn_shift + j * 64, ka, a2, a3);
+            }
             if (p.b_kmajor) {
-              tma_load_4d(sb, tb, full_bar(s), kbb, n0 + sg.b_mn_shift, b2, b3);
+              tma_load_4d_pair(sb, tb, fb, kbb, nb0, b2, b3);
             } else {
-#pragma unroll
-              for (int j = 0; j < C::BN_S / 64; ++j) tma_load_4d(sb + j * (BK * 128), tb, full_bar(s), n0 + sg.b_mn_shift + j * 64, kbb, b2, b3);
-            }
-          } else {
-            constexpr int HB = BN / MC;
-            if (p.b_kmajor) {
-              tma_load_4d_mc(sb + crank * (HB * 128), tb, full_bar(s), kbb, n0 + sg.b_mn_shift + crank * HB, b2, b3, (uint16_t)((1 << MC) - 1));
+  #pragma unroll
+              for (int j = 0; j < C::BN_S / 64; ++j) tma_load_4d_pair(sb + j * (BK * 128), tb, fb, nb0 + j * 64, kbb, b2, b3);
+            }
+          } else if (leader) {
+            mbar_expect_tx(full_bar(s), tx_bytes);
+            const uint32_t sa = smem_base + s * C::STAGE_BYTES;
+            const uint32_t sb = sa + A_STAGE_BYTES;
+            const CUtensorMap* ta = &p.tmA[sg.a_idx];
+            const CUtensorMap* tb = &p.tmB[sg.b_idx];
+            const int bz2 = sg.rep_is_batch ? (sg.rep_c2_0 + rep) : z2;
+            const int a2 = p.a_batched[sg.a_idx] ? bz2 : 0, a3 = p.a_batched[sg.a_idx] ? z3 : 0;
+            const int b2 = p.b_batched[sg.b_idx] ? bz2 : 0, b3 = p.b_batched[sg.b_idx] ? z3 : 0;
+            const int ka = sg.a_k0 + kb * BK, kbb = sg.b_k0 + z2 * sg.b_k0_z2 + kb * BK;
+            if (p.a_kmajor) {
+              tma_load_4d(sa, ta, full_bar(s), ka, m0 + sg.a_mn_shift, a2, a3);
             } else {
-#pragma unroll
-              for (int j = 0; j < HB / 64; ++j) {
-                const int jj = crank * (HB / 64) + j;
-                tma_load_4d_mc(sb + jj * (BK * 128), tb, full_bar(s), n0 + sg.b_mn_shift + jj * 64, kbb, b2, b3, (uint16_t)((1 << MC) - 1));
-              }
-            }
-          }
+  #pragma unroll
+              for (int j = 0; j < BM / 64; ++j) tma_load_4d(sa + j * (BK * 128), ta, full_bar(s), m0 + sg.a_mn_shift + j * 64, ka, a2, a3);
+            }
+            if (MC == 1) {
+              if (p.b_kmajor) {
+                tma_load_4d(sb, tb, full_bar(s), kbb, n0 + sg.b_mn_shift, b2, b3);
+              } else {
+  #pragma unroll
+                for (int j = 0; j < C::BN_S / 64; ++j) tma_load_4d(sb + j * (BK * 128), tb, full_bar(s), n0 + sg.b_mn_shift + j * 64, kbb, b2, b3);
+              }
+            } else {
+              constexpr int HB = BN / MC;
+              if (p.b_kmajor) {
+                tma_load_4d_mc(sb + crank * (HB * 128), tb, full_bar(s), kbb, n0 + sg.b_mn_shift + crank * HB, b2, b3, (uint16_t)((1 << MC) - 1));
+              } else {
+  #pragma unroll
+                for (int j = 0; j < HB / 64; ++j) {
+                  const int jj = crank * (HB / 64) + j;
+                  tma_load_4d_mc(sb + jj * (BK * 128), tb, full_bar(s), n0 + sg.b_mn_shift + jj * 64, kbb, b2, b3, (uint16_t)((1 << MC) - 1));
+                }
+              }
+            }
+          }
+          const int nkb = (sg.nk + BK - 1) / BK;
+          if (++kb == nkb) {
+            kb = 0;
+            if (++rep == sg.nrep) {
+              rep = 0;
+              ++seg;
+            }
+          }
+          if (++s == C::STAGES) s = 0, ph ^= 1;
         }
-        const int nkb = (sg.nk + BK - 1) / BK;
-        if (++kb == nkb) {
-          kb = 0;
-          if (++rep == sg.nrep) {
-            rep = 0;
-            ++seg;
-          }
-        }
-        if (++s == C::STAGES) s = 0, ph ^= 1;
       }
+      if (!next_unit(j, unit)) break;
     }
   } else if (warp == 1 && (!PAIR || crank == 0)) {
     const bool leader = elect_one();
@@ -287,36 +310,41 @@
     int s = 0;
     uint32_t ph = 0;
     int segi = 0;
-    while (sched.next(tile, it_begin, it_end)) {
-      const int acc = segi & 1;
-      mbar_wait(tmem_empty_bar(acc), ((segi >> 1) & 1) ^ 1);
-      asm volatile("tcgen05.fence::after_thread_sync;" ::: "memory");
-      const uint32_t dcol = tmem_base + (uint32_t)(acc * BN);
-      for (int it = it_begin; it < it_end; ++it) {
-        mbar_wait(full_bar(s), ph);
+    int unit = first_unit;
+    for (int j = 0;; ++j) {
+      UnitWalk walk(p, unit);
+      while (walk.next(p, tile, it_begin, it_end)) {
+        const int acc = segi & 1;
+        mbar_wait(tmem_empty_bar(acc), ((segi >> 1) & 1) ^ 1);
         asm volatile("tcgen05.fence::after_thread_sync;" ::: "memory");
-        if (leader) {
-          const uint64_t ad = adesc0 + (uint64_t)(s * (C::STAGE_BYTES >> 4));
-          const uint64_t bd = bdesc0 + (uint64_t)(s * (C::STAGE_BYTES >> 4));
-          if constexpr (PAIR) {
-#pragma unroll
-            for (int k = 0; k < BK / 16; ++k)
-              umma_f16_pair(dcol, ad + (uint64_t)(k * a_kstep), bd + (uint64_t)(k * b_kstep), idesc, (it > it_begin || k > 0) ? 1u : 0u);
-            umma_commit_pair(empty_bar(s), (uint16_t)3);
-            if (it == it_end - 1) umma_commit_pair(tmem_full_bar(acc), (uint16_t)3);
-          } else {
-#pragma unroll
-            for (int k = 0; k < BK / 16; ++k)
-              umma_f16(dcol, ad + (uint64_t)(k * a_kstep), bd + (uint64_t)(k * b_kstep), idesc, (it > it_begin || k > 0) ? 1u : 0u);
-            if (MC == 1) umma_commit(empty_bar(s));
-            else umma_commit_mc(empty_bar(s), (uint16_t)((1 << MC) - 1));
-            if (it == it_end - 1) umma_commit(tmem_full_bar(acc));
-          }
+        const uint32_t dcol = tmem_base + (uint32_t)(acc * BN);
+        for (int it = it_begin; it < it_end; ++it) {
+          mbar_wait(full_bar(s), ph);
+          asm volatile("tcgen05.fence::after_thread_sync;" ::: "memory");
+          if (leader) {
+            const uint64_t ad = adesc0 + (uint64_t)(s * (C::STAGE_BYTES >> 4));
+            const uint64_t bd = bdesc0 + (uint64_t)(s * (C::STAGE_BYTES >> 4));
+            if constexpr (PAIR) {
+  #pragma unroll
+              for (int k = 0; k < BK / 16; ++k)
+                umma_f16_pair(dcol, ad + (uint64_t)(k * a_kstep), bd + (uint64_t)(k * b_kstep), idesc, (it > it_begin || k > 0) ? 1u : 0u);
+              umma_commit_pair(empty_bar(s), (uint16_t)3);
+              if (it == it_end - 1) umma_commit_pair(tmem_full_bar(acc), (uint16_t)3);
+            } else {
+  #pragma unroll
+              for (int k = 0; k < BK / 16; ++k)
+                umma_f16(dcol, ad + (uint64_t)(k * a_kstep), bd + (uint64_t)(k * b_kstep), idesc, (it > it_begin || k > 0) ? 1u : 0u);
+              if (MC == 1) umma_commit(empty_bar(s));
+              else umma_commit_mc(empty_bar(s), (uint16_t)((1 << MC) - 1));
+              if (it == it_end - 1) umma_commit(tmem_full_bar(acc));
+            }
+          }
+          __syncwarp();
+          if (++s == C::STAGES) s = 0, ph ^= 1;
         }
-        __syncwarp();
-        if (++s == C::STAGES) s = 0, ph ^= 1;
+        ++segi;
       }
-      ++segi;
+      if (!next_unit(j, unit)) break;
     }
   } else if (warp >= 2) {
     const uint32_t tmem_empty_leader0 = PAIR ? mapa_u32(tmem_empty_bar(0), 0) : 0;
@@ -338,244 +366,249 @@
     int segi = 0;
     int pc = 0;
     int staged_n0 = -1, staged_z2 = -1;
-    while (sched.next(tile, it_begin, it_end)) {
-      int m0, n0, z2, z3;
-      decode(tile, m0, n0, z2, z3);
-      const int acc = segi & 1;
-      if (!p.out_t && (n0 != staged_n0 || (p.bias_z2 != nullptr && z2 != staged_z2))) {
-        asm volatile("bar.sync 1, %0;" ::"n"(ET) : "memory");
-        const float* bz = p.bias_z2 ? p.bias_z2 + (long long)z2 * p.bz2_stride : nullptr;
-        for (int j = et; j < BN; j += ET) {
-          const int n = n0 + j;
-          float bsum = 0.f;
-          if (n < p.N) {
-            if (p.bias) bsum += __ldg(p.bias + n);
-            if (bz) bsum += __ldg(bz + n);
-          }
-          sbias[j] = bsum;
+    int unit = first_unit;
+    for (int j = 0;; ++j) {
+      UnitWalk walk(p, unit);
+      while (walk.next(p, tile, it_begin, it_end)) {
+        int m0, n0, z2, z3;
+        decode(tile, m0, n0, z2, z3);
+        const int acc = segi & 1;
+        if (!p.out_t && (n0 != staged_n0 || (p.bias_z2 != nullptr && z2 != staged_z2))) {
+          asm volatile("bar.sync 1, %0;" ::"n"(ET) : "memory");
+          const float* bz = p.bias_z2 ? p.bias_z2 + (long long)z2 * p.bz2_stride : nullptr;
+          for (int j = et; j < BN; j += ET) {
+            const int n = n0 + j;
+            float bsum = 0.f;
+            if (n < p.N) {
+              if (p.bias) bsum += __ldg(p.bias + n);
+              if (bz) bsum += __ldg(bz + n);
+            }
+            sbias[j] = bsum;
+          }
+          asm volatile("bar.sync 1, %0;" ::"n"(ET) : "memory");
+          staged_n0 = n0;
+          staged_z2 = z2;
         }
-        asm volatile("bar.sync 1, %0;" ::"n"(ET) : "memory");
-        staged_n0 = n0;
-        staged_z2 = z2;
-      }
-      const uint32_t tbase = tmem_base + ((uint32_t)(q * 32) << 16) + (uint32_t)(acc * BN);
-      const uint32_t full_parity = (segi >> 1) & 1;
-      if (p.out_dtype == PT_OUT_BF16) {
-        constexpr int CH = C::EPI_COLS;
-        constexpr int NPASS = BN / CH;
-        constexpr int NPH = (NPASS + ES - 1) / ES;
-        constexpr int VPR = CH / 8;
-        constexpr int RPI = 32 / VPR;
-        constexpr int NIT = 32 / RPI;
-        uint8_t* stg_base = sepi + ew * (C::EPI_BUFS * 32 * CH * 2);
-        uint8_t* stg = stg_base + (pc & (C::EPI_BUFS - 1)) * (32 * CH * 2);
-        auto cell = [&](int row, int chunk) { return stg + row * (CH * 2) + ((chunk ^ ((row >> 1) & 3)) << 4); };
-        const int mw = m0 + q * 32;
-        const int crow = lane / VPR, cvec = lane % VPR;
-        const long long zoff_r = (long long)z2 * p.rsz2 + (long long)z3 * p.rsz3;
-        const bool has_res = p.res != nullptr;
-        const int last_c = min(NPASS, (p.N - n0 + CH - 1) / CH) - 1;
-        const int last_k = last_c >= half ? (last_c - half) / ES : -1;
-        uint32_t v[2][CH];
-        bf16x8 rr[2][NIT];
-        auto load_res = [&](int pass, bf16x8* dst) {
-          if (p.out_t) {
-            const int mb = mw + cvec * 8;
-#pragma unroll
+        const uint32_t tbase = tmem_base + ((uint32_t)(q * 32) << 16) + (uint32_t)(acc * BN);
+        const uint32_t full_parity = (segi >> 1) & 1;
+        if (p.out_dtype == PT_OUT_BF16) {
+          constexpr int CH = C::EPI_COLS;
+          constexpr int NPASS = BN / CH;
+          constexpr int NPH = (NPASS + ES - 1) / ES;
+          constexpr int VPR = CH / 8;
+          constexpr int RPI = 32 / VPR;
+          constexpr int NIT = 32 / RPI;
+          uint8_t* stg_base = sepi + ew * (C::EPI_BUFS * 32 * CH * 2);
+          uint8_t* stg = stg_base + (pc & (C::EPI_BUFS - 1)) * (32 * CH * 2);
+          auto cell = [&](int row, int chunk) { return stg + row * (CH * 2) + ((chunk ^ ((row >> 1) & 3)) << 4); };
+          const int mw = m0 + q * 32;
+          const int crow = lane / VPR, cvec = lane % VPR;
+          const long long zoff_r = (long long)z2 * p.rsz2 + (long long)z3 * p.rsz3;
+          const bool has_res = p.res != nullptr;
+          const int last_c = min(NPASS, (p.N - n0 + CH - 1) / CH) - 1;
+          const int last_k = last_c >= half ? (last_c - half) / ES : -1;
+          uint32_t v[2][CH];
+          bf16x8 rr[2][NIT];
+          auto load_res = [&](int pass, bf16x8* dst) {
+            if (p.out_t) {
+              const int mb = mw + cvec * 8;
+  #pragma unroll
+              for (int i = 0; i < NIT; ++i) {
+                const int n = n0 + pass * CH + crow + i * RPI;
+                if (n < p.N && mb < p.M) dst[i] = ld16(p.res + zoff_r + (long long)n * p.rsm + mb);
+              }
+              return;
+            }
+            const int nb = n0 + pass * CH + cvec * 8;
+  #pragma unroll
             for (int i = 0; i < NIT; ++i) {
-              const int n = n0 + pass * CH + crow + i * RPI;
-              if (n < p.N && mb < p.M) dst[i] = ld16(p.res + zoff_r + (long long)n * p.rsm + mb);
-            }
-            return;
-          }
-          const int nb = n0 + pass * CH + cvec * 8;
-#pragma unroll
-          for (int i = 0; i < NIT; ++i) {
-            const int m = mw + crow + i * RPI;
-            if (m < p.M && nb < p.N) dst[i] = ld16(p.res + zoff_r + (long long)m * p.rsm + nb);
-          }
-        };
-        float brow = 0.f;
-        if (p.out_t && mw + lane < p.M) {
-          if (p.bias) brow += __ldg(p.bias + mw + lane);
-          if (p.bias_z2) brow += __ldg(p.bias_z2 + (long long)z2 * p.bz2_stride + mw + lane);
-        }
-        if (has_res && last_k >= 0) load_res(half, rr[0]);
-        mbar_wait(tmem_full_bar(acc), full_parity);
-        asm volatile("tcgen05.fence::after_thread_sync;" ::: "memory");
-        if (last_k < 0) {
-          release_acc(acc);
-        } else {
-          tmem_ld32(tbase + (uint32_t)(half * CH), v[0]);
-        }
-#pragma unroll
-        for (int k = 0; k < NPH; ++k) {
-          const int c = half + k * ES;
-          const int nb = n0 + c * CH;
-          if (k <= last_k) {
-            __syncwarp();
-            asm volatile("tcgen05.wait::ld.sync.aligned;" ::: "memory");
-            if (k < last_k) {
-              tmem_ld32(tbase + (uint32_t)((c + ES) * CH), v[(k + 1) & 1]);
-              if (has_res) load_res(c + ES, rr[(k + 1) & 1]);
-            } else {
-              release_acc(acc);
-            }
-            stg = stg_base + (pc & (C::EPI_BUFS - 1)) * (32 * CH * 2);
-            if (lane == 0) {
-              if (C::EPI_BUFS == 2) asm volatile("cp.async.bulk.wait_group.read 1;" ::: "memory");
-              else asm volatile("cp.async.bulk.wait_group.read 0;" ::: "memory");
-            }
-            __syncwarp();
-            if (has_res) {
-#pragma unroll
-              for (int i = 0; i < NIT; ++i) st16(cell(crow + i * RPI, cvec), rr[k & 1][i]);
+              const int m = mw + crow + i * RPI;
+              if (m < p.M && nb < p.N) dst[i] = ld16(p.res + zoff_r + (long long)m * p.rsm + nb);
+            }
+          };
+          float brow = 0.f;
+          if (p.out_t && mw + lane < p.M) {
+            if (p.bias) brow += __ldg(p.bias + mw + lane);
+            if (p.bias_z2) brow += __ldg(p.bias_z2 + (long long)z2 * p.bz2_stride + mw + lane);
+          }
+          if (has_res && last_k >= 0) load_res(half, rr[0]);
+          mbar_wait(tmem_full_bar(acc), full_parity);
+          asm volatile("tcgen05.fence::after_thread_sync;" ::: "memory");
+          if (last_k < 0) {
+            release_acc(acc);
+          } else {
+            tmem_ld32(tbase + (uint32_t)(half * CH), v[0]);
+          }
+  #pragma unroll
+          for (int k = 0; k < NPH; ++k) {
+            const int c = half + k * ES;
+            const int nb = n0 + c * CH;
+            if (k <= last_k) {
               __syncwarp();
-            }
-            if (p.out_t) {
-#pragma unroll
-              for (int j = 0; j < CH; ++j) {
-                bf16* cellp = reinterpret_cast<bf16*>(cell(j, lane >> 3)) + (lane & 7);
-                float f = fmaf(__uint_as_float(v[k & 1][j]), p.alpha, brow);
-                if (has_res) f += __bfloat162float(*cellp);
-                *cellp = __float2bfloat16_rn(f);
+              asm volatile("tcgen05.wait::ld.sync.aligned;" ::: "memory");
+              if (k < last_k) {
+                tmem_ld32(tbase + (uint32_t)((c + ES) * CH), v[(k + 1) & 1]);
+                if (has_res) load_res(c + ES, rr[(k + 1) & 1]);
+              } else {
+                release_acc(acc);
+              }
+              stg = stg_base + (pc & (C::EPI_BUFS - 1)) * (32 * CH * 2);
+              if (lane == 0) {
+                if (C::EPI_BUFS == 2) asm volatile("cp.async.bulk.wait_group.read 1;" ::: "memory");
+                else asm volatile("cp.async.bulk.wait_group.read 0;" ::: "memory");
+              }
+              __syncwarp();
+              if (has_res) {
+  #pragma unroll
+                for (int i = 0; i < NIT; ++i) st16(cell(crow + i * RPI, cvec), rr[k & 1][i]);
+                __syncwarp();
+              }
+              if (p.out_t) {
+  #pragma unroll
+                for (int j = 0; j < CH; ++j) {
+                  bf16* cellp = reinterpret_cast<bf16*>(cell(j, lane >> 3)) + (lane & 7);
+                  float f = fmaf(__uint_as_float(v[k & 1][j]), p.alpha, brow);
+                  if (has_res) f += __bfloat162float(*cellp);
+                  *cellp = __float2bfloat16_rn(f);
+                }
+                fence_proxy_async_smem();
+                __syncwarp();
+                if (lane == 0) {
+                  tma_store_4d(&p.tmO, smem_u32(stg), mw, nb, z2, z3);
+                  tma_store_commit();
+                }
+                ++pc;
+                continue;
+              }
+              const float* sb = sbias + c * CH;
+  #pragma unroll
+              for (int g = 0; g < VPR; ++g) {
+                const float4 b0 = *reinterpret_cast<const float4*>(sb + g * 8), b1 = *reinterpret_cast<const float4*>(sb + g * 8 + 4);
+                const float bs[8] = {b0.x, b0.y, b0.z, b0.w, b1.x, b1.y, b1.z, b1.w};
+                float f[8];
+  #pragma unroll
+                for (int j = 0; j < 8; ++j) f[j] = fmaf(__uint_as_float(v[k & 1][g * 8 + j]), p.alpha, bs[j]);
+                uint8_t* mine = cell(lane, g);
+                if (has_res) {
+                  const bf16x8 t = ld16(mine);
+  #pragma unroll
+                  for (int h = 0; h < 4; ++h) {
+                    const float2 u = bf2_to_f2(t.w[h]);
+                    f[2 * h] += u.x;
+                    f[2 * h + 1] += u.y;
+                  }
+                }
+                bf16x8 t;
+  #pragma unroll
+                for (int h = 0; h < 4; ++h) t.w[h] = f2_to_bf2(f[2 * h], f[2 * h + 1]);
+                st16(mine, t);
               }
               fence_proxy_async_smem();
               __syncwarp();
               if (lane == 0) {
-                tma_store_4d(&p.tmO, smem_u32(stg), mw, nb, z2, z3);
+                tma_store_4d(&p.tmO, smem_u32(stg), nb, mw, z2, z3);
                 tma_store_commit();
               }
               ++pc;
-              continue;
-            }
-            const float* sb = sbias + c * CH;
-#pragma unroll
-            for (int g = 0; g < VPR; ++g) {
-              const float4 b0 = *reinterpret_cast<const float4*>(sb + g * 8), b1 = *reinterpret_cast<const float4*>(sb + g * 8 + 4);
-              const float bs[8] = {b0.x, b0.y, b0.z, b0.w, b1.x, b1.y, b1.z, b1.w};
-              float f[8];
-#pragma unroll
-              for (int j = 0; j < 8; ++j) f[j] = fmaf(__uint_as_float(v[k & 1][g * 8 + j]), p.alpha, bs[j]);
-              uint8_t* mine = cell(lane, g);
-              if (has_res) {
-                const bf16x8 t = ld16(mine);
-#pragma unroll
-                for (int h = 0; h < 4; ++h) {
-                  const float2 u = bf2_to_f2(t.w[h]);
-                  f[2 * h] += u.x;
-                  f[2 * h + 1] += u.y;
-                }
-              }
-              bf16x8 t;
-#pragma unroll
-              for (int h = 0; h < 4; ++h) t.w[h] = f2_to_bf2(f[2 * h], f[2 * h + 1]);
-              st16(mine, t);
-            }
-            fence_proxy_async_smem();
-            __syncwarp();
-            if (lane == 0) {
-              tma_store_4d(&p.tmO, smem_u32(stg), nb, mw, z2, z3);
-              tma_store_commit();
-            }
-            ++pc;
-          }
-        }
-      } else {
-        const int m = m0 + q * 32 + lane;
-        const bool m_ok = m < p.M;
-        const long long out_off = (long long)z2 * p.osz2 + (long long)z3 * p.osz3 + (long long)m * p.osm;
-        constexpr int FC = C::F32_COLS;
-        constexpr int NCH = BN / FC;
-        constexpr int NPH = (NCH + ES - 1) / ES;
-        const int last_c = min(NCH, (p.N - n0 + FC - 1) / FC) - 1;
-        const int last_k = last_c >= half ? (last_c - half) / ES : -1;
-        uint32_t v[2][FC];
-        mbar_wait(tmem_full_bar(acc), full_parity);
-        asm volatile("tcgen05.fence::after_thread_sync;" ::: "memory");
-        if (last_k < 0) {
-          release_acc(acc);
+            }
+          }
         } else {
-          tmem_ld16(tbase + (uint32_t)(half * FC), v[0]);
-        }
-        float* tile = reinterpret_cast<float*>(sepi) + ew * (32 * (FC + 1));
-        const int mrow0 = m0 + q * 32;
-        const long long zoff = (long long)z2 * p.osz2 + (long long)z3 * p.osz3;
-#pragma unroll
-        for (int k = 0; k < NPH; ++k) {
-          const int c = half + k * ES;
-          const int nb = n0 + c * FC;
-          if (k <= last_k) {
-            __syncwarp();
-            asm volatile("tcgen05.wait::ld.sync.aligned;" ::: "memory");
-            if (k < last_k) {
-              tmem_ld16(tbase + (uint32_t)((c + ES) * FC), v[(k + 1) & 1]);
-            } else {
-              release_acc(acc);
-            }
-            float f[FC];
-#pragma unroll
-            for (int j = 0; j < FC; ++j) f[j] = fmaf(__uint_as_float(v[k & 1][j]), p.alpha, sbias[c * FC + j]);
-            if (p.out_dtype == PT_OUT_F32) {
-              if (m_ok) {
-                float* o = reinterpret_cast<float*>(p.out) + out_off + nb;
-#pragma unroll
-                for (int g = 0; g < FC / 4; ++g) {
-                  if (nb + g * 4 + 4 <= p.N) {
-                    *reinterpret_cast<float4*>(o + g * 4) = make_float4(f[g * 4], f[g * 4 + 1], f[g * 4 + 2], f[g * 4 + 3]);
-                  } else {
-#pragma unroll
-                    for (int j = 0; j < 4; ++j)
-                      if (nb + g * 4 + j < p.N) o[g * 4 + j] = f[g * 4 + j];
-                  }
-                }
-              }
-            } else if (p.vec_red) {
-              float* vt = reinterpret_cast<float*>(sepi) + ew * (32 * FC);
-#pragma unroll
-              for (int g = 0; g < FC / 4; ++g)
-                *reinterpret_cast<float4*>(vt + lane * FC + ((g ^ ((lane >> 1) & 3)) << 2)) = make_float4(f[g * 4], f[g * 4 + 1], f[g * 4 + 2], f[g * 4 + 3]);
+          const int m = m0 + q * 32 + lane;
+          const bool m_ok = m < p.M;
+          const long long out_off = (long long)z2 * p.osz2 + (long long)z3 * p.osz3 + (long long)m * p.osm;
+          constexpr int FC = C::F32_COLS;
+          constexpr int NCH = BN / FC;
+          constexpr int NPH = (NCH + ES - 1) / ES;
+          const int last_c = min(NCH, (p.N - n0 + FC - 1) / FC) - 1;
+          const int last_k = last_c >= half ? (last_c - half) / ES : -1;
+          uint32_t v[2][FC];
+          mbar_wait(tmem_full_bar(acc), full_parity);
+          asm volatile("tcgen05.fence::after_thread_sync;" ::: "memory");
+          if (last_k < 0) {
+            release_acc(acc);
+          } else {
+            tmem_ld16(tbase + (uint32_t)(half * FC), v[0]);
+          }
+          float* tile = reinterpret_cast<float*>(sepi) + ew * (32 * (FC + 1));
+          const int mrow0 = m0 + q * 32;
+          const long long zoff = (long long)z2 * p.osz2 + (long long)z3 * p.osz3;
+  #pragma unroll
+          for (int k = 0; k < NPH; ++k) {
+            const int c = half + k * ES;
+            const int nb = n0 + c * FC;
+            if (k <= last_k) {
               __syncwarp();
-              const int c4 = lane & 3, rsub = lane >> 2;
-              const int n = nb + c4 * 4;
-              if (n < p.N) {
-                float* o = reinterpret_cast<float*>(p.out) + zoff + n;
-#pragma unroll
-                for (int it = 0; it < 4; ++it) {
-                  const int r = it * 8 + rsub;
-                  if (mrow0 + r < p.M) {
-                    const float4 t = *reinterpret_cast<const float4*>(vt + r * FC + ((c4 ^ ((r >> 1) & 3)) << 2));
-                    float* dst = o + (long long)(mrow0 + r) * p.osm;
-                    if (n + 4 <= p.N) {
-                      asm volatile("red.global.add.v4.f32 [%0], {%1, %2, %3, %4};" ::"l"(dst), "f"(t.x), "f"(t.y), "f"(t.z), "f"(t.w) : "memory");
+              asm volatile("tcgen05.wait::ld.sync.aligned;" ::: "memory");
+              if (k < last_k) {
+                tmem_ld16(tbase + (uint32_t)((c + ES) * FC), v[(k + 1) & 1]);
+              } else {
+                release_acc(acc);
+              }
+              float f[FC];
+  #pragma unroll
+              for (int j = 0; j < FC; ++j) f[j] = fmaf(__uint_as_float(v[k & 1][j]), p.alpha, sbias[c * FC + j]);
+              if (p.out_dtype == PT_OUT_F32) {
+                if (m_ok) {
+                  float* o = reinterpret_cast<float*>(p.out) + out_off + nb;
+  #pragma unroll
+                  for (int g = 0; g < FC / 4; ++g) {
+                    if (nb + g * 4 + 4 <= p.N) {
+                      *reinterpret_cast<float4*>(o + g * 4) = make_float4(f[g * 4], f[g * 4 + 1], f[g * 4 + 2], f[g * 4 + 3]);
                     } else {
-                      const float tv[4] = {t.x, t.y, t.z, t.w};
-#pragma unroll
+  #pragma unroll
                       for (int j = 0; j < 4; ++j)
-                        if (n + j < p.N) atomicAdd(dst + j, tv[j]);
+                        if (nb + g * 4 + j < p.N) o[g * 4 + j] = f[g * 4 + j];
                     }
                   }
                 }
-              }
-              __syncwarp();
-            } else {
-#pragma unroll
-              for (int j = 0; j < FC; ++j) tile[lane * (FC + 1) + j] = f[j];
-              __syncwarp();
-              const int col = lane % FC, rsub = lane / FC;
-              const int n = nb + col;
-              if (n < p.N) {
-                float* o = reinterpret_cast<float*>(p.out) + zoff + (long long)n * p.osn;
-#pragma unroll 8
-                for (int r = rsub; r < 32; r += 32 / FC) {
-                  if (mrow0 + r < p.M) atomicAdd(o + (long long)(mrow0 + r) * p.osm, tile[r * (FC + 1) + col]);
+              } else if (p.vec_red) {
+                float* vt = reinterpret_cast<float*>(sepi) + ew * (32 * FC);
+  #pragma unroll
+                for (int g = 0; g < FC / 4; ++g)
+                  *reinterpret_cast<float4*>(vt + lane * FC + ((g ^ ((lane >> 1) & 3)) << 2)) = make_float4(f[g * 4], f[g * 4 + 1], f[g * 4 + 2], f[g * 4 + 3]);
+                __syncwarp();
+                const int c4 = lane & 3, rsub = lane >> 2;
+                const int n = nb + c4 * 4;
+                if (n < p.N) {
+                  float* o = reinterpret_cast<float*>(p.out) + zoff + n;
+  #pragma unroll
+                  for (int it = 0; it < 4; ++it) {
+                    const int r = it * 8 + rsub;
+                    if (mrow0 + r < p.M) {
+                      const float4 t = *reinterpret_cast<const float4*>(vt + r * FC + ((c4 ^ ((r >> 1) & 3)) << 2));
+                      float* dst = o + (long long)(mrow0 + r) * p.osm;
+                      if (n + 4 <= p.N) {
+                        asm volatile("red.global.add.v4.f32 [%0], {%1, %2, %3, %4};" ::"l"(dst), "f"(t.x), "f"(t.y), "f"(t.z), "f"(t.w) : "memory");
+                      } else {
+                        const float tv[4] = {t.x, t.y, t.z, t.w};
+  #pragma unroll
+                        for (int j = 0; j < 4; ++j)
+                          if (n + j < p.N) atomicAdd(dst + j, tv[j]);
+                      }
+                    }
+                  }
                 }
+                __syncwarp();
+              } else {
+  #pragma unroll
+                for (int j = 0; j < FC; ++j) tile[lane * (FC + 1) + j] = f[j];
+                __syncwarp();
+                const int col = lane % FC, rsub = lane / FC;
+                const int n = nb + col;
+                if (n < p.N) {
+                  float* o = reinterpret_cast<float*>(p.out) + zoff + (long long)n * p.osn;
+  #pragma unroll 8
+                  for (int r = rsub; r < 32; r += 32 / FC) {
+                    if (mrow0 + r < p.M) atomicAdd(o + (long long)(mrow0 + r) * p.osm, tile[r * (FC + 1) + col]);
+                  }
+                }
               }
             }
           }
         }
+        ++segi;
       }
-      ++segi;
+      if (!next_unit(j, unit)) break;
     }
     if (lane == 0) tma_store_wait_all();
   }
@@ -670,19 +703,6 @@
     attr[0].val.clusterDim.z = 1;
     cfg.attrs = attr;
     cfg.numAttrs = 1;
-    static int max_clusters = 0;
-    if (!max_clusters) {
-      int n = 0;
-      cudaLaunchConfig_t q = cfg;
-      q.gridDim = dim3((unsigned)(pt_num_sms_physical() / MC * MC), 1, 1);
-      if (cudaOccupancyMaxActiveClusters(&n, gemm_kernel<BN, MC, PAIR>, &q) != cudaSuccess || n < 1) {
-        (void)cudaGetLastError();
-        n = pt_num_sms_physical() / MC;
-      }
-      max_clusters = n;
-      if (getenv("PT_GEMM_DEBUG")) fprintf(stderr, "[pt_gemm] BN=%d cluster=%d pair=%d: %d clusters resident at once\n", BN, MC, (int)PAIR, n);
-    }
-    if ((int)grid.x / MC > max_clusters) cfg.gridDim = dim3((unsigned)(max_clusters * MC), 1, 1);
     PT_CUDA_OK(cudaLaunchKernelEx(&cfg, gemm_kernel<BN, MC, PAIR>, kp));
   }
   PT_LAUNCH_CHECK();
@@ -821,9 +841,7 @@
   PT_REQUIRE(tiles * total < (1ll << 31), "pt_gemm: work space too large");
   kp.mt = (int)mtg;
   kp.nt = (int)nt;
-  kp.tiles = (int)tiles;
   kp.work = (int)(tiles * total);
-  kp.streamk = streamk ? 1 : 0;
   {
     static const bool no_group = getenv("PT_GEMM_NO_GROUP") != nullptr;
     const long long resident = (long long)sms * (bn <= 128 ? 2 : 1) / mc;
@@ -852,10 +870,16 @@
                 g->out_stride_z3 % 4 == 0 && (reinterpret_cast<uintptr_t>(g->out) & 15) == 0 && !getenv("PT_GEMM_SCALAR_RED"))
                    ? 1 : 0;
 
-  const long long slots = (long long)sms * (bn <= 128 ? 2 : 1) / mc;
-  long long G = streamk ? (kp.work / 4 > 0 ? kp.work / 4 : 1) : tiles;
-  if (G > slots) G = slots;
-  dim3 grid((unsigned)(G * mc), 1, 1);
+  constexpr int SK_UNITS_PER_SLOT = 2;
+  const long long slots = (long long)sms * (bn <= 128 ? 2 : 1);
+  long long unit_iters = total;
+  if (streamk) {
+    unit_iters = (kp.work + SK_UNITS_PER_SLOT * slots - 1) / (SK_UNITS_PER_SLOT * slots);
+    if (unit_iters < 4) unit_iters = 4;
+  }
+  kp.unit_iters = (int)unit_iters;
+  const long long units = (kp.work + unit_iters - 1) / unit_iters;
+  dim3 grid((unsigned)(units * mc), 1, 1);
   cudaStream_t st = reinterpret_cast<cudaStream_t>(stream);
   g_last_tile = bn | (bn == 256 && mc == 1 ? 1 : 0);
   switch (bn) {
diff --git a/prompt_tts_b200/csrc/tc_common.cuh b/prompt_tts_b200/csrc/tc_common.cuh
--- a/prompt_tts_b200/csrc/tc_common.cuh
+++ b/prompt_tts_b200/csrc/tc_common.cuh
@@ -133,6 +133,27 @@
   asm volatile("mov.u32 %0, %%cluster_ctarank;" : "=r"(r));
   return r;
 }
+template <bool MULTICAST>
+__device__ __forceinline__ void clc_try_cancel(uint32_t resp, uint32_t bar) {
+  if constexpr (MULTICAST)
+    asm volatile("clusterlaunchcontrol.try_cancel.async.shared::cta.mbarrier::complete_tx::bytes.multicast::cluster::all.b128 [%0], [%1];"
+                 ::"r"(resp), "r"(bar) : "memory");
+  else
+    asm volatile("clusterlaunchcontrol.try_cancel.async.shared::cta.mbarrier::complete_tx::bytes.b128 [%0], [%1];" ::"r"(resp), "r"(bar) : "memory");
+}
+__device__ __forceinline__ int clc_first_ctaid_x(uint32_t resp) {
+  uint32_t ok, x;
+  asm volatile(
+      "{\n\t.reg .pred p;\n\t.reg .b128 r;\n\t"
+      "ld.shared.b128 r, [%2];\n\t"
+      "clusterlaunchcontrol.query_cancel.is_canceled.pred.b128 p, r;\n\t"
+      "selp.u32 %0, 1, 0, p;\n\t"
+      "clusterlaunchcontrol.query_cancel.get_first_ctaid::x.b32.b128 %1, r;\n\t}"
+      : "=r"(ok), "=r"(x)
+      : "r"(resp)
+      : "memory");
+  return ok ? (int)x : -1;
+}
 __device__ __forceinline__ void cluster_sync_all() {
   asm volatile("barrier.cluster.arrive.release.aligned;" ::: "memory");
   asm volatile("barrier.cluster.wait.acquire.aligned;" ::: "memory");
diff --git a/prompt_tts_b200/engine.py b/prompt_tts_b200/engine.py
--- a/prompt_tts_b200/engine.py
+++ b/prompt_tts_b200/engine.py
@@ -22,26 +22,31 @@
 
 class SideLane:
 
+    CAP_BYTES = 2 << 30
+
     def __init__(self, device):
         self.stream = torch.cuda.Stream(device)
         self.keep: List[torch.Tensor] = []
+        self.kept_bytes = 0
         self.dirty = False
 
-    def run(self, fn: Callable[[], None], keep: Sequence[torch.Tensor] = ()) -> None:
+    def run(self, fn: Callable[[], None], keep: Sequence[torch.Tensor] = (), grads: Sequence[torch.Tensor] = ()) -> None:
         self.stream.wait_stream(torch.cuda.current_stream())
         with torch.cuda.stream(self.stream):
             fn()
         self.keep.extend(keep)
+        self.keep.extend(grads)
+        self.kept_bytes += sum(g.numel() * g.element_size() for g in grads)
         self.dirty = True
+        if self.kept_bytes > self.CAP_BYTES:
+            self.join()
 
     def join(self) -> None:
         if self.dirty:
             torch.cuda.current_stream().wait_stream(self.stream)
             self.dirty = False
             self.keep.clear()
-
-
-SIDE_LANE = os.environ.get("PT_SIDE_LANE", "0") == "1"
+            self.kept_bytes = 0
 
 
 class PackCache:
@@ -161,13 +166,13 @@
     def pgrad_conv(self, p: torch.Tensor) -> torch.Tensor:
         return self._grad_buf([p], "conv")
 
+    def side(self, fn: Callable[[], None], keep: Sequence[torch.Tensor], grads: Sequence[torch.Tensor]) -> None:
+        if self.cache.lane is None:
+            self.cache.lane = SideLane(grads[0].device)
+        self.cache.lane.run(fn, keep=keep, grads=grads)
+
     def side_colsum(self, x2d: torch.Tensor, out: torch.Tensor) -> None:
-        if not SIDE_LANE or not x2d.is_cuda:
-            ops.colsum(x2d, out)
-            return
-        if self.cache.lane is None:
-            self.cache.lane = SideLane(x2d.device)
-        self.cache.lane.run(lambda: ops.colsum(x2d, out, lite=True), keep=(x2d, out))
+        self.side(lambda: ops.colsum(x2d, out, lite=True), keep=(out,), grads=(x2d,))
 
     def join_side(self) -> None:
         if self.cache.lane is not None:
@@ -199,8 +204,11 @@
         v.owned = True
 
 
-def _wgrad_gemm(dy2d_op, x2d_op, seg, N: int, K: int, out: torch.Tensor, out_stride_m: int) -> None:
-    ops.gemm([dy2d_op], [x2d_op], [seg], N, K, out, out_strides=(out_stride_m, 0, 0), out_mode=OUT_F32_ATOMIC_ADD)
+def _wgrad_gemm(tape: Tape, dy2: torch.Tensor, x2: torch.Tensor, N: int, K: int, out: torch.Tensor) -> None:
+    M = x2.shape[0]
+    tape.side(lambda: ops.gemm([ops.operand(dy2, False)], [ops.operand(x2, False)], [ops.segment(M)], N, K, out, out_strides=(K, 0, 0),
+                               out_mode=OUT_F32_ATOMIC_ADD),
+              keep=(x2, out), grads=(dy2,))
 
 
 def linear(tape: Tape, x: Var, wparams: Sequence[torch.Tensor], bias: Optional[Sequence[torch.Tensor]] = None,
@@ -227,7 +235,7 @@
         if bias is not None:
             tape.side_colsum(dy2, tape.pgrad_cat(bias) if len(bias) > 1 else tape.pgrad(bias[0]))
         gw = (tape.pgrad_cat(wparams) if len(wparams) > 1 else tape.pgrad(wparams[0])).view(N, K)
-        _wgrad_gemm(ops.operand(dy2, False), ops.operand(x2, False), ops.segment(M), N, K, gw, K)
+        _wgrad_gemm(tape, dy2, x2, N, K, gw)
         if x.needs_grad:
             dx = torch.empty_like(x2) if (x.grad is None or not x.owned) else x.grad.reshape(M, K)
             prev = x.grad.reshape(M, K) if x.grad is not None else None
@@ -292,17 +300,21 @@
         if tshift is not None and tshift.dproj is not None:
             ops.batch_colsum(dy, tshift.dproj[:, tshift.offset:], tshift.dproj.stride(0))
         g3 = tape.pgrad_conv(wparam)
-        dy_op = ops.operand(dy, False, batched=True)
-        if stride == 1:
-            seg = ops.segment(Lo, b_k0=-1, b_k0_z2=1, nrep=B, rep_is_batch=True)
-            ops.gemm([dy_op], [ops.operand(xd, False, batched=True)], [seg], Co, Ci, g3, out_strides=(3 * Ci, Ci, 0), nz2=3,
-                     out_mode=OUT_F32_ATOMIC_ADD)
-        else:
-            for t, (ai, sh) in enumerate(taps):
-                xs = xd[:, 0::2] if ai == 0 else xd[:, 1::2]
-                seg = ops.segment(Lo, b_k0=sh, nrep=B, rep_is_batch=True)
-                ops.gemm([dy_op], [ops.operand(xs, False, batched=True)], [seg], Co, Ci, g3[:, t],
-                         out_strides=(3 * Ci, 0, 0), out_mode=OUT_F32_ATOMIC_ADD)
+
+        def wgrad():
+            dy_op = ops.operand(dy, False, batched=True)
+            if stride == 1:
+                seg = ops.segment(Lo, b_k0=-1, b_k0_z2=1, nrep=B, rep_is_batch=True)
+                ops.gemm([dy_op], [ops.operand(xd, False, batched=True)], [seg], Co, Ci, g3, out_strides=(3 * Ci, Ci, 0), nz2=3,
+                         out_mode=OUT_F32_ATOMIC_ADD)
+            else:
+                for t, (ai, sh) in enumerate(taps):
+                    xs = xd[:, 0::2] if ai == 0 else xd[:, 1::2]
+                    seg = ops.segment(Lo, b_k0=sh, nrep=B, rep_is_batch=True)
+                    ops.gemm([dy_op], [ops.operand(xs, False, batched=True)], [seg], Co, Ci, g3[:, t],
+                             out_strides=(3 * Ci, 0, 0), out_mode=OUT_F32_ATOMIC_ADD)
+
+        tape.side(wgrad, keep=(xd, g3), grads=(dy,))
         if x.needs_grad:
             dy_k = ops.operand(dy, True, batched=True)
             wp_mn = ops.operand(wp, False)
```

Measured after the change: 527,700 (median of 6 runs). -1.1%, worse.
